# OettlM/STEDM

Measured on AMD Instinct MI355X. Metric: U-Net denoising steps/sec (32x32x4 latent, bs=64), higher is better.
Workload: dtype f16; 1 GPU; HER2-style DDIM-50 + CFG 1.5 (rescale 0.7) denoising step, NS32 U-Net (234.6M params, random-init PRNG weights), 32x32x4 latents + 3-ch layout concat, style vector 512; batch_per_gpu=64, global_batch=64, latent=32x32x4, cfg=cond+uncond per step, parallelism=dp1 (independent latents, no in-loop collective)

## Files before the change

include/stedm_hip.h:

```cpp
#ifndef STEDM_HIP_H
#define STEDM_HIP_H

#include <stdint.h>

#ifdef __cplusplus
extern "C" {
#endif

#define STEDM_ABI_VERSION 31

#define STEDM_F16 0
#define STEDM_BF16 1

#define STEDM_CONV_S1 0
#define STEDM_CONV_DOWN 1
#define STEDM_CONV_UP 2
#define STEDM_CONV_UP_SUBPIXEL 3
#define STEDM_CONV_S2D 4

int stedm_abi_version(void);
const char* stedm_last_error(void);
int stedm_device_cus(void);

#define STEDM_F16G_RAW 1
// ... 38 lines not shown
                           const float* gamma, const float* beta, float eps, int groups, int act, int B, int HW,
                           void* out_hi, void* out_lo, void* raw_hi, void* raw_lo, float* mean_rstd, const float* film, long film_bstride,
                           int film_off, int mm_dtype, void* stream);
int stedm_gn_apply16c_x16(int c1, const float* cs1, int nslab1, const float* x2, int c2, const float* cs2, int nslab2, int x2_bmod,
                          const float* gamma, const float* beta, float eps, int groups, int act, int B, int HW,
                          void* out_hi, void* raw_hi, int mm_dtype, void* stream);
int stedm_avgpool2x2(const float* in, float* out, int B, int H, int W, int C, float* chan_stats, int nslab, void* stream);
int stedm_replicate2x2(const float* in, float* out, int B, int H, int W, int C, float scale, int accumulate, float* chan_stats, int nslab,
                       void* stream);
int stedm_gn_apply16c_resample(const float* x, int C, const float* cs, int nslab, const float* gamma, const float* beta, float eps, int groups,
                               int act, int B, int H, int W, int mode, void* out_hi, void* out_lo, float* xr, float* mean_rstd, int mm_dtype,
                               void* stream);
int stedm_gn_stats(const float* x1, int c1, const float* x2, int c2, int x2_bmod, int groups, int B, int HW,
                   double* stats, void* stream);
int stedm_gn_apply16(const float* x1, int c1, const float* x2, int c2, int x2_bmod, const float* gamma,
                     const float* beta, float eps, int groups, int act, const double* stats, int B, int HW,
                     void* out_hi, void* out_lo, int mm_dtype, void* stream);

typedef struct stedm_conv_args {
  const float* src1;
  const float* src2;
  int32_t c1, c2, src2_bmod;
  int32_t B, Hin, Win;
  int32_t mode;
  int32_t ks;
  const float* scale;
  const float* shift;
  int32_t act;
  const void* w_hi;
  const void* w_lo;
  const float* bias;
  const float* emb;
  int32_t emb_bstride;
  const float* res;
  float* out;
  int32_t cout;
  int32_t npass;
  int32_t mm_dtype;
  const void* src16_hi;
  const void* src16_lo;
  int32_t act_out;
  void* out16_hi;
  void* out16_lo;
  const void* w_frag;
  float* chan_stats;
  const void* src16b_hi;
  const void* w_frag_b;
  const float* bias_b;
  int32_t cb;
  float* ws;
  int64_t ws_floats;
  int32_t chan_nslab;
  const void* w_frag16;
  const void* w_frag_b16;
  int32_t pad_br;
  const float* gn_gamma;
  const float* gn_beta;
  float gn_eps;
  int32_t gn_groups;
  int32_t gn_act;
  void* gn_out16;
  float* gn_mr;
  int32_t gn_only;
  void* gn_out16_lo;
  void* qkv_q;
  void* qkv_k;
  void* qkv_vt;
  int32_t qkv_T, qkv_Tp, qkv_heads;
  float qkv_qscale;
  const float* ln_gamma;
  const float* ln_beta;
  const float* ln_res;
  float ln_eps;
  int32_t out16_stride;
  void* gn_coop;
  const uint32_t* gn_coop_epoch;
  uint32_t* gn_coop_tmo;
  int32_t src16_cstride;
  int32_t k_chan0;
  int32_t w_cin;
  int32_t res_bmod;
  const float* res2;
  int32_t ws_bmod;
} stedm_conv_args;
int stedm_conv_igemm(const stedm_conv_args* args, void* stream);
int stedm_conv_fused_skip_ok(const stedm_conv_args* args);
int stedm_conv3x3_tiles_ok(int Hout, int Wout);
int stedm_im2col_rows16(const void* src16, void* dst16, int B, int Hs, int Ws, int C, int mode, void* stream);
int stedm_conv_rs_ok(const stedm_conv_args* args);
int stedm_conv_partials(const stedm_conv_args* args, int32_t* nshare, int dry, void* stream);
int stedm_conv_finish(const stedm_conv_args* args, int nshare, void* stream);

int stedm_conv_in(const float* x1, int c1, const float* x2, int c2, int x2_bmod, const float* w_oihw,
                  const float* bias, float* out, int B, int H, int W, int cout, float* chan_stats, void* stream);
int stedm_conv_out(const float* src, int c, const float* chan_stats, int nslab, const float* gamma, const float* beta,
                   float eps, int groups, const float* w_hwio, const float* bias, float* out, int B, int H, int W,
                   int cout, void* stream);

int stedm_time_embed(const int64_t* t, const float* freqs, const float* w0t, const float* b0,
                     const float* w2t, const float* b2, float* emb, float* ws, int B, int mc, int ted,
                     void* stream);
int stedm_time_embed_f32(const float* t, const float* freqs, const float* w0t, const float* b0,
                         const float* w2t, const float* b2, float* emb, float* ws, int B, int mc, int ted,
                         void* stream);
int stedm_emb_proj(const float* emb, const float* wt, const float* bias, float* out, int B, int k, int ntot,
                   void* stream);

int stedm_linear(const float* x, const float* wt, const float* bias, float* out, int B, int k, int n, int act_in,
                 int act_out, void* stream);

int stedm_attn_legacy(const float* qkv, float* out, int B, int T, int heads, int ch, void* stream);
int stedm_attn_legacy16(const void* qkv, int qkv_is16, void* out16, int B, int T, int heads, int ch, int mm_dtype, void* stream);
#define STEDM_ATTN_HEADS_FIRST 0
#define STEDM_ATTN_QKV_FIRST 1
int stedm_attn_qkv(const float* qkv, float* out, int B, int T, int heads, int ch, int order, void* stream);
int stedm_attn_qkv16(const void* qkv, int qkv_is16, void* out16, int B, int T, int heads, int ch, int mm_dtype, int order, void* stream);

int stedm_ddim_step(const float* x, const float* e_c, const float* e_u, const float* noise,
                    const float* coefs, const int32_t* step_idx, float cfg_scale, float rescale_phi,
                    float* x_prev, float* pred_x0, int B, int C, int H, int W, void* stream);
int stedm_ddim_step_ex(const float* x, const float* e_c, const float* e_u, const float* noise, const float* coefs, const int32_t* step_idx,
                       int n_iters, float cfg_scale, float rescale_phi, int draw, float temperature, float noise_dropout, long first_id,
                       unsigned long long seed, float* x_prev, float* pred_x0, float* eps_out, float* noise_out, int B, int C, int H, int W,
                       void* stream);
int stedm_ddim_step_rows(const float* x, const float* e_c, const float* e_u, const float* noise, const float* coefs,
                         const int32_t* step_idx, int n_iters, const float* scales, float rescale_phi, int draw, long first_id,
                         unsigned long long seed, float* x_prev, float* pred_x0, int B, int C, int H, int W, void* stream);
int stedm_step_advance(int32_t* step_idx, int delta, void* stream);
int stedm_step_set_t(const int64_t* ts_table, const int32_t* step_idx, int64_t* t_buf, int B, void* stream);
int stedm_step_set_t_f32(const float* ts_table, const int32_t* step_idx, float* t_buf, int B, void* stream);

#define STEDM_DPM_NCOEF 6
int stedm_dpm_step(float* x, const float* e_c, const float* e_u, float* x0_prev, float* pred_x0, const float* coefs,
                   const int32_t* step_idx, float cfg_scale, long n, void* stream);

#define STEDM_DPMU_NCOEF 24
#define STEDM_DPMU_ALL 0
#define STEDM_DPMU_MODEL 1
#define STEDM_DPMU_COMBINE 2
int stedm_dpm_update(float* x, float* base, const float* e_c, const float* e_u, float* slots, long slot_stride, float* pred_x0,
                     const float* rows, const int32_t* step_idx, float cfg_scale, int mode, long n, void* stream);
int stedm_dpm_threshold(float* slots, long slot_stride, const float* rows, const int32_t* step_idx, float max_val, int B, long n,
                        float* q_out, void* stream);

#define STEDM_PLMS_EULER 0
#define STEDM_PLMS_HEUN 1
#define STEDM_PLMS_MULTISTEP 2
int stedm_plms_step(float* x, const float* e_c, const float* e_u, float* ring, const float* coefs, const int32_t* step_idx,
                    int n_iters, int phase, float cfg_scale, float* pred_x0, float* x_tmp, long n, void* stream);

int stedm_svit_patch_embed(const float* img, int B, int ns, int H, int W, int patch, const float* ln_w,
                           const float* ln_b, float eps, const float* wt, const float* bias, const float* pos,
                           const float* cls, float* x, int dim, void* stream);
int stedm_svit_patch_ln16(const float* img, int B, int ns, int H, int W, int patch, const float* ln_w, const float* ln_b,
                          float eps, void* out_hi, void* out_lo, int mm_dtype, void* stream);
int stedm_svit_tok_place(const float* tok, const float* pos, const float* cls, float* x, int B, int ntok, int dim, void* stream);
int stedm_ln_apply16(const float* x, const float* gamma, const float* beta, float eps, void* out_hi, void* out_lo,
                     long rows, int dim, int mm_dtype, void* stream);
int stedm_qkv_pack(const void* qkv, int qkv_is16, float qscale, void* q_hi, void* q_lo, void* k_hi, void* k_lo, void* vt_hi,
                   void* vt_lo, int B, int T, int Tp, int heads, int mm_dtype, void* stream);
int stedm_lsa_flash(const void* q_hi, const void* q_lo, const void* k_hi, const void* k_lo, const void* vt_hi,
                    const void* vt_lo, void* out_hi, void* out_lo, int B, int T, int Tp, int heads, int npass,
                    int mm_dtype, void* stream);
int stedm_qkv_pack_mx8(const void* qkv, int qkv_is16, float qscale, void* q8, void* qs, void* k8, void* ks, void* vt8, void* vs, int B, int T,
                       int Tp, int heads, int mm_dtype, void* stream);
int stedm_lsa_flash_mx8(const void* q8, const void* qs, const void* k8, const void* ks, const void* vt8, const void* vs, void* out16, int B,
// ... 179 lines not shown
```

stedm_amd/_lib.py:

```python
from __future__ import annotations

import ctypes as C
import os

_HERE = os.path.dirname(os.path.abspath(__file__))
LIB_PATH = os.environ.get("STEDM_HIP_LIB") or os.path.join(_HERE, "libstedm_hip.so")

ABI_VERSION = 31
F16, BF16 = 0, 1
CONV_S1, CONV_DOWN, CONV_UP, CONV_UP_SUBPIXEL, CONV_S2D = 0, 1, 2, 3, 4
STREAM_POSTERIOR = 0x40000


class StedmHipError(RuntimeError):
    pass


class ConvArgs(C.Structure):
    _fields_ = [
        ("src1", C.c_void_p), ("src2", C.c_void_p),
        ("c1", C.c_int32), ("c2", C.c_int32), ("src2_bmod", C.c_int32),
        ("B", C.c_int32), ("Hin", C.c_int32), ("Win", C.c_int32),
        ("mode", C.c_int32), ("ks", C.c_int32),
        ("scale", C.c_void_p), ("shift", C.c_void_p),
        ("act", C.c_int32),
        ("w_hi", C.c_void_p), ("w_lo", C.c_void_p), ("bias", C.c_void_p),
        ("emb", C.c_void_p), ("emb_bstride", C.c_int32),
        ("res", C.c_void_p), ("out", C.c_void_p),
        ("cout", C.c_int32), ("npass", C.c_int32), ("mm_dtype", C.c_int32),
        ("src16_hi", C.c_void_p), ("src16_lo", C.c_void_p),
        ("act_out", C.c_int32), ("out16_hi", C.c_void_p), ("out16_lo", C.c_void_p),
        ("w_frag", C.c_void_p), ("chan_stats", C.c_void_p),
        ("src16b_hi", C.c_void_p), ("w_frag_b", C.c_void_p), ("bias_b", C.c_void_p), ("cb", C.c_int32),
        ("ws", C.c_void_p), ("ws_floats", C.c_int64), ("chan_nslab", C.c_int32), ("w_frag16", C.c_void_p), ("w_frag_b16", C.c_void_p), ("pad_br", C.c_int32),
        ("gn_gamma", C.c_void_p), ("gn_beta", C.c_void_p), ("gn_eps", C.c_float), ("gn_groups", C.c_int32), ("gn_act", C.c_int32), ("gn_out16", C.c_void_p), ("gn_mr", C.c_void_p), ("gn_only", C.c_int32),
        ("gn_out16_lo", C.c_void_p),
        ("qkv_q", C.c_void_p), ("qkv_k", C.c_void_p), ("qkv_vt", C.c_void_p),
        ("qkv_T", C.c_int32), ("qkv_Tp", C.c_int32), ("qkv_heads", C.c_int32), ("qkv_qscale", C.c_float),
        ("ln_gamma", C.c_void_p), ("ln_beta", C.c_void_p), ("ln_res", C.c_void_p), ("ln_eps", C.c_float),
        ("out16_stride", C.c_int32),
        ("gn_coop", C.c_void_p), ("gn_coop_epoch", C.c_void_p), ("gn_coop_tmo", C.c_void_p),
        ("src16_cstride", C.c_int32), ("k_chan0", C.c_int32), ("w_cin", C.c_int32), ("res_bmod", C.c_int32),
        ("res2", C.c_void_p), ("ws_bmod", C.c_int32),
    ]


_P, _I, _F = C.c_void_p, C.c_int, C.c_float
SIGNATURES = {
    "stedm_abi_version": (_I, []),
    "stedm_last_error": (C.c_char_p, []),
    "stedm_device_cus": (_I, []),
    "stedm_f16_guard_set": (_I, [_P]),
    "stedm_pack_conv_weight": (_I, [_P, _P, _P, _I, _I, _I, _I, _P]),
    "stedm_pack_conv_weight_up": (_I, [_P, _P, _P, _I, _I, _I, _P]),
    "stedm_pack_conv_weight_frag": (_I, [_P, _P, _I, _I, _I, _I, _P]),
    "stedm_pack_conv_weight_up_frag": (_I, [_P, _P, _I, _I, _I, _P]),
    "stedm_pack_conv_weight_frag16": (_I, [_P, C.c_long, C.c_long, _I, _P, _I, _I, _I, _I, _P]),
    "stedm_pack_conv_weight_frag16_hl": (_I, [_P, C.c_long, C.c_long, _I, _P, _I, _I, _I, _P]),
    "stedm_pack_conv_weight_frag16_hl1": (_I, [_P, C.c_long, C.c_long, _I, _P, _I, _I, _I, _P]),
    "stedm_pack_conv_weight_up_frag16_hl": (_I, [_P, _P, _I, _I, _I, _P]),
    "stedm_pack_conv_weight_s2d_frag16_hl": (_I, [_P, _P, _I, _I, _I, _I, _P]),
    "stedm_pack_conv_weight_s2d_frag": (_I, [_P, _P, _I, _I, _I, _I, _P]),
    "stedm_space_to_depth16": (_I, [_P, _I, _I, _I, _I, _P, _P, _I, _P]),
    "stedm_transpose_f32": (_I, [_P, _P, _I, _I, _P]),
    "stedm_gn_scale_shift": (_I, [_P, _I, _P, _I, _I, _P, _P, _F, _I, _I, _I, _P, _P, _P]),
    "stedm_gn_nslab": (_I, [_I, _I]),
    "stedm_gn_stats": (_I, [_P, _I, _P, _I, _I, _I, _I, _I, _P, _P]),
    "stedm_gn_apply16": (_I, [_P, _I, _P, _I, _I, _P, _P, _F, _I, _I, _P, _I, _I, _P, _P, _I, _P]),
    "stedm_gn_chan_nslab": (_I, [_I]),
    "stedm_gn_chan_stats": (_I, [_P, _I, _I, _I, _I, _P, _P]),
    "stedm_gn_chan_stats16": (_I, [_P, _I, _I, _I, _I, _P, _P, _P, _I, _P]),
    "stedm_gn_apply16c": (_I, [_P, _I, _P, _I, _P, _I, _P, _I, _I, _P, _P, _F, _I, _I, _I, _I, _P, _P, _P, _P, _I, _P]),
    "stedm_gn_apply16c_mr": (_I, [_P, _I, _P, _I, _P, _I, _P, _I, _I, _P, _P, _F, _I, _I, _I, _I, _P, _P, _P, _P, _P, _I, _P]),
    "stedm_conv3x3_tiles_ok": (_I, [_I, _I]),
    "stedm_im2col_rows16": (_I, [_P, _P, _I, _I, _I, _I, _I, _P]),
    "stedm_philox_normal": (_I, [_P, _I, _I, _P, _I, C.c_ulonglong, C.c_uint, _P]),
    "stedm_ddim_mask_blend": (_I, [_P, _P, _P, C.c_long, C.c_long, _P, _P, _P, _P, _P, _I, _I, _I, C.c_long, C.c_ulonglong, _P]),
    "stedm_ddpm_step": (_I, [_P, _P, _P, _P, _I, _I, _P, _P, C.c_long, C.c_long, _P, _P, _P, _P, _I, _I, _I, C.c_long,
                            C.c_ulonglong, C.c_ulonglong, _P]),
    "stedm_ddpm_step_ex": (_I, [_P, _P, _P, _P, _P, _I, _I, _P, _P, _F, _P, _I, _P, C.c_long, C.c_long, _P, _P, _P, _P, _P, _P, _P, _P,
                               _I, _I, _I, C.c_long, C.c_ulonglong, C.c_ulonglong, _P]),
    "stedm_gn_apply16c_film": (_I, [_P, _I, _P, _I, _P, _I, _P, _I, _I, _P, _P, _F, _I, _I, _I, _I, _P, _P, _P, _P, _P, _P, C.c_long, _I, _I, _P]),
    "stedm_gn_apply16c_drop": (_I, [_P, _I, _P, _I, _P, _I, _P, _I, _I, _P, _P, _F, _I, _I, _I, _I, _P, _P, _P, _P, _P, _I, _F, C.c_ulonglong, C.c_uint,
                                    C.c_uint, _P, _P]),
    "stedm_gn_apply16c_film_drop": (_I, [_P, _I, _P, _I, _P, _I, _P, _I, _I, _P, _P, _F, _I, _I, _I, _I, _P, _P, _P, _P, _P, _P, C.c_long, _I, _I, _F,
                                         C.c_ulonglong, C.c_uint, C.c_uint, _P, _P]),
    "stedm_gn_apply16c_x16": (_I, [_I, _P, _I, _P, _I, _P, _I, _I, _P, _P, _F, _I, _I, _I, _I, _P, _P, _I, _P]),
    "stedm_conv_igemm": (_I, [C.POINTER(ConvArgs), _P]),
    "stedm_conv_fused_skip_ok": (_I, [C.POINTER(ConvArgs)]),
    "stedm_conv_rs_ok": (_I, [C.POINTER(ConvArgs)]),
    "stedm_conv_partials": (_I, [C.POINTER(ConvArgs), C.POINTER(C.c_int32), _I, _P]),
    "stedm_conv_finish": (_I, [C.POINTER(ConvArgs), _I, _P]),
    "stedm_conv_in": (_I, [_P, _I, _P, _I, _I, _P, _P, _P, _I, _I, _I, _I, _P, _P]),
    "stedm_conv_out": (_I, [_P, _I, _P, _I, _P, _P, _F, _I, _P, _P, _P, _I, _I, _I, _I, _P]),
    "stedm_time_embed": (_I, [_P, _P, _P, _P, _P, _P, _P, _P, _I, _I, _I, _P]),
    "stedm_time_embed_f32": (_I, [_P, _P, _P, _P, _P, _P, _P, _P, _I, _I, _I, _P]),
    "stedm_emb_proj": (_I, [_P, _P, _P, _P, _I, _I, _I, _P]),
    "stedm_linear": (_I, [_P, _P, _P, _P, _I, _I, _I, _I, _I, _P]),
    "stedm_attn_legacy": (_I, [_P, _P, _I, _I, _I, _I, _P]),
    "stedm_attn_legacy16": (_I, [_P, _I, _P, _I, _I, _I, _I, _I, _P]),
    "stedm_attn_qkv": (_I, [_P, _P, _I, _I, _I, _I, _I, _P]),
    "stedm_attn_qkv16": (_I, [_P, _I, _P, _I, _I, _I, _I, _I, _I, _P]),
    "stedm_ddim_step": (_I, [_P, _P, _P, _P, _P, _P, _F, _F, _P, _P, _I, _I, _I, _I, _P]),
    "stedm_ddim_step_ex": (_I, [_P, _P, _P, _P, _P, _P, _I, _F, _F, _I, _F, _F, C.c_long, C.c_ulonglong, _P, _P, _P, _P, _I, _I, _I, _I,
                               _P]),
    "stedm_ddim_step_rows": (_I, [_P, _P, _P, _P, _P, _P, _I, _P, _F, _I, C.c_long, C.c_ulonglong, _P, _P, _I, _I, _I, _I, _P]),
    "stedm_step_advance": (_I, [_P, _I, _P]),
    "stedm_step_set_t": (_I, [_P, _P, _P, _I, _P]),
    "stedm_step_set_t_f32": (_I, [_P, _P, _P, _I, _P]),
    "stedm_dpm_step": (_I, [_P, _P, _P, _P, _P, _P, _P, _F, C.c_long, _P]),
    "stedm_dpm_update": (_I, [_P, _P, _P, _P, _P, C.c_long, _P, _P, _P, _F, _I, C.c_long, _P]),
    "stedm_dpm_threshold": (_I, [_P, C.c_long, _P, _P, _F, _I, C.c_long, _P, _P]),
    "stedm_plms_step": (_I, [_P, _P, _P, _P, _P, _P, _I, _I, _F, _P, _P, C.c_long, _P]),
    "stedm_svit_patch_embed": (_I, [_P, _I, _I, _I, _I, _I, _P, _P, _F, _P, _P, _P, _P, _P, _I, _P]),
    "stedm_svit_patch_ln16": (_I, [_P, _I, _I, _I, _I, _I, _P, _P, _F, _P, _P, _I, _P]),
    "stedm_svit_tok_place": (_I, [_P, _P, _P, _P, _I, _I, _I, _P]),
    "stedm_ln_apply16": (_I, [_P, _P, _P, _F, _P, _P, C.c_long, _I, _I, _P]),
    "stedm_qkv_pack": (_I, [_P, _I, _F, _P, _P, _P, _P, _P, _P, _I, _I, _I, _I, _I, _P]),
    "stedm_lsa_flash": (_I, [_P, _P, _P, _P, _P, _P, _P, _P, _I, _I, _I, _I, _I, _I, _P]),
    "stedm_lsa_flash_drop": (_I, [_P, _P, _P, _P, _P, _P, _P, _P, _I, _I, _I, _I, _I, _I, _F, C.c_ulonglong, C.c_uint, _P]),
    "stedm_dropout_rows": (_I, [_P, _P, _P, _P, _P, C.c_long, _F, C.c_ulonglong, C.c_uint, _I, _P]),
    "stedm_qkv_pack_mx8": (_I, [_P, _I, _F, _P, _P, _P, _P, _P, _P, _I, _I, _I, _I, _I, _P]),
    "stedm_lsa_flash_mx8": (_I, [_P, _P, _P, _P, _P, _P, _P, _I, _I, _I, _I, _I, _P]),
    "stedm_svit_head": (_I, [_P, _I, _I, _I, _I, _P, _P, _P, _F, _P, _P, _P, _I, _P, C.c_long, _P]),
    "stedm_lsa_bwd_ws_floats": (C.c_long, [_I, _I, _I, _I]),
    "stedm_lsa_bwd16_ws_bytes": (C.c_long, [_I, _I, _I, _I, _F]),
# ... 123 lines not shown
```

stedm_amd/csrc/conv_dma_bf16_p1.hip:

```cpp
#include "conv_igemm_dma9.inc"
#include "conv_rs.inc"
namespace stedm {
int conv_dma_pick_bf16_p1(ConvParams& p, hipStream_t st, bool dry) {
  int rc = conv_rs_pick<__bf16>(p, st, dry);
  if (rc >= 0 || dry || p.a.src16b_hi || p.a.mode == STEDM_CONV_S2D || p.a.qkv_q || p.a.ln_gamma) return rc;
  if (p.a.src16_cstride || p.a.k_chan0 || p.a.w_cin || p.a.res_bmod || p.a.res2 || p.partials || p.a.out16_stride) return rc;
  rc = dma9_pick<__bf16>(p, st);
  return rc >= 0 ? rc : dma_pick<1, __bf16>(p, st);
}
}

extern "C" int stedm_debug_conv_stamps(unsigned long long* host_out, int nblocks) {
  if (!host_out || nblocks <= 0 || nblocks > 2048) { stedm::set_error("debug_conv_stamps: bad args"); return 1; }
  hipError_t e = hipMemcpyFromSymbol(host_out, HIP_SYMBOL(g_conv_stamps), (size_t)nblocks * 8 * sizeof(unsigned long long));
  if (e != hipSuccess) { stedm::set_error("debug_conv_stamps: %s", hipGetErrorString(e)); return 2; }
  return 0;
}
```

stedm_amd/csrc/conv_dma_f16_p1.hip:

```cpp
#include "conv_igemm_dma9.inc"
#include "conv_rs.inc"
namespace stedm {
int conv_dma_pick_f16_p1(ConvParams& p, hipStream_t st, bool dry) {
  int rc = conv_rs_pick<_Float16>(p, st, dry);
  if (rc >= 0 || dry || p.a.src16b_hi || p.a.mode == STEDM_CONV_S2D || p.a.qkv_q || p.a.ln_gamma) return rc;
  if (p.a.src16_cstride || p.a.k_chan0 || p.a.w_cin || p.a.res_bmod || p.a.res2 || p.partials || p.a.out16_stride) return rc;
  rc = dma9_pick<_Float16>(p, st);
  return rc >= 0 ? rc : dma_pick<1, _Float16>(p, st);
}
int conv_splitk_finish(ConvParams& p, int nshare, hipStream_t st) { return splitk_finish_impl(p, nshare, st); }
}
```

stedm_amd/csrc/conv_igemm_dma.hip:

```cpp
#include "conv_common.hpp"
using namespace stedm;

namespace stedm {
int conv_dma_pick_f16_p1(ConvParams&, hipStream_t, bool dry);
int conv_dma_pick_f16_p3(ConvParams&, hipStream_t, bool dry);
int conv_dma_pick_bf16_p1(ConvParams&, hipStream_t, bool dry);
int conv_dma_pick_bf16_p3(ConvParams&, hipStream_t, bool dry);
}

int stedm::conv_launch_dma(ConvParams& p, hipStream_t st, bool dry) {
  const stedm_conv_args& a = p.a;
  if (a.src16b_hi && a.npass != 1) { set_error("conv_igemm(dma): the fused skip phase is single-product only"); return 1; }
  if (dry && a.npass != 1 && !a.w_frag16) return 1;
  if (a.src16b_hi && ((long)a.B * a.Hin * a.Win * a.cb >= (1L << 31) || a.cb * 2 + 256 > STEDM_ZERO_PAGE_BYTES)) {
    set_error("conv_igemm(dma): fused skip operand too large (cb=%d)", a.cb);
    return 1;
  }
  if ((long)a.B * a.Hin * a.Win * (p.cstride > p.Cin ? p.cstride : p.Cin) >= (1L << 31)) {
    set_error("conv_igemm(dma): activation tensor too large for 32-bit element offsets");
    return 1;
  }
  if (p.Cin * 2 + 256 > STEDM_ZERO_PAGE_BYTES) { set_error("conv_igemm(dma): Cin too large for the zero page"); return 1; }
  const bool f16 = a.mm_dtype == STEDM_F16;
  int rc = a.npass == 3 ? (f16 ? conv_dma_pick_f16_p3(p, st, dry) : conv_dma_pick_bf16_p3(p, st, dry))
                        : (f16 ? conv_dma_pick_f16_p1(p, st, dry) : conv_dma_pick_bf16_p1(p, st, dry));
  if (dry) return rc < 0 ? 1 : 0;
  if (rc < 0 && a.ln_gamma) { set_error("conv_igemm(dma): the register-streamed kernel does not run this LayerNorm-epilogue problem (see stedm_conv_rs_ok)"); return 1; }
  if (rc < 0 && a.qkv_q) { set_error("conv_igemm(dma): the register-streamed kernel does not run this qkv-epilogue problem (see stedm_conv_rs_ok)"); return 1; }
  if (rc < 0 && (a.src16_cstride || a.k_chan0 || a.w_cin || a.res_bmod || a.res2 || p.partials || a.out16_stride)) {
    set_error("conv_igemm(dma): the register-streamed kernel does not run this problem, and no other kernel knows a K window, res_bmod / res2, the partials-only form or out16_stride (see stedm_conv_rs_ok)");
    return 1;
  }
  if (rc < 0 && a.src16b_hi) { set_error("conv_igemm(dma): no kernel runs this fused skip problem (see stedm_conv_fused_skip_ok)"); return 1; }
  if (rc < 0) { set_error("conv_igemm(dma): no tile configuration fits (Hin=%d Win=%d mode=%d Cin=%d)", a.Hin, a.Win, a.mode, p.Cin); return 1; }
  return rc;
}
```

stedm_amd/csrc/conv_rs.inc:

```
#pragma once
#include <type_traits>

#include "conv_igemm_dma.inc"
#include "gn_fold.hpp"

static __device__ unsigned long long g_conv_stamps[2048 * 8];
#define STAMP(K) if (STEDM_DBG(p.dbg, 1024) && tid == 0 && blockIdx.x < 2048) g_conv_stamps[blockIdx.x * 8 + (K)] = wall_clock64()
#define STAMPC(K) if (STEDM_DBG(p.dbg, 1024) && tid == 0 && blockIdx.x < 2048) g_conv_stamps[blockIdx.x * 8 + (K)] = __builtin_amdgcn_s_memtime()

#ifdef STEDM_CONV_DIAG
#define RS_DIAG(BIT) ((STEDM_CONV_DIAG) & (BIT))
#else
#define RS_DIAG(BIT) 0
#endif

__device__ __forceinline__ float rs_lane_xor1(float v) {
  return __builtin_bit_cast(float, __builtin_amdgcn_mov_dpp(__builtin_bit_cast(int, v), 0xB1, 0xF, 0xF, true));
}
template <typename T>
__device__ __forceinline__ unsigned rs_pack2(float lo, float hi) {
  typedef T V2T __attribute__((ext_vector_type(2)));
  V2T v; v[0] = (T)lo; v[1] = (T)hi;
  return __builtin_bit_cast(unsigned, v);
}
// ... 204 lines not shown
    }                                                                          \
  }
   \
   \
#define LOAD_A3(BASE, TAP, F)                                                  \
  {                                                                            \
    unsigned a_, a2_;                                                          \
    asm volatile("v_add_u32 %0, %1, %2" : "=v"(a_) : "s"((BASE) + tapd[TAP]), "v"(aofs[F]));             \
    asm volatile("v_add_u32 %0, %1, %2" : "=v"(a2_) : "s"((BASE) + tapd[TAP] + a_half), "v"(aofs[F]));   \
    LDSR(ah[(F) & (NAR - 1)], a_);                                             \
    LDSR(al[(F) & (NAR - 1)], a2_);                                            \
  }
#define A3_AFTER(Q, WHAT)                                                                                          \
  {                                                                                                                \
    if ((Q) + 2 < 8) { WHAT(Acur, t, (Q) + 2) }                                                                    \
    else if (t + 1 < NS) { WHAT(Acur, t + 1, (Q) + 2 - 8) }                                                         \
    else { WHAT(Anext, 0, (Q) + 2 - 8) }                                                                           \
  }
#define A3_ADDR_HI(BASE, TAP, F) asm volatile("v_add_u32 %0, %1, %2" : "=v"(a_) : "s"((BASE) + tapd[TAP]), "v"(aofs[F]));
#define A3_ADDR_LO(BASE, TAP, F) asm volatile("v_add_u32 %0, %1, %2" : "=v"(a2_) : "s"((BASE) + tapd[TAP] + a_half), "v"(aofs[F]));
#define RS3_CHUNK(PAR)                                                                                             \
  _Pragma("unroll") for (int u = 0; u < NU; ++u) {                                                                 \
    const int t = u >> 1, hf = u & 1, sb = (t & 1) ^ (PAR);                                                        \
    if (u == NU - 1) __builtin_amdgcn_s_barrier();    \
    _Pragma("unroll") for (int i = 0; i < 4; ++i) {                                                                \
      const int R = hf * 4 + i;                             \
      _Pragma("unroll") for (int m = 0; m < 12; ++m) {                                                             \
        const int j = m & 3;                                                                                       \
        __builtin_amdgcn_sched_barrier(0);                                                                         \
        if (m < 4) acc[R][j] = MM<T>::mfma16(al[R & (NAR - 1)], bh[sb][j], acc[R][j]);                              \
        else if (m < 8) acc[R][j] = MM<T>::mfma16(ah[R & (NAR - 1)], bl[sb][j], acc[R][j]);                         \
        else acc[R][j] = MM<T>::mfma16(ah[R & (NAR - 1)], bh[sb][j], acc[R][j]);                                    \
        __builtin_amdgcn_sched_barrier(0);                                                                         \
        if (m == 0) { LDSR(ah[(R + 1) & (NAR - 1)], a_); }                                                          \
        else if (m == 1) { LDSR(al[(R + 1) & (NAR - 1)], a2_); }                                                    \
        if (R == 0 && m >= 4) {                                                                                    \
                        \
          if (m == 4) { int g_ = g0 + t + 1; g_ = g_ < gmax ? g_ : gmax; wcur = wq + ((size_t)(unsigned)g_ << 13) + voff; } \
          if (m < 8) bh[sb ^ 1][m - 4] = *reinterpret_cast<const V8*>(wcur + (m - 4) * 1024);                        \
          else bl[sb ^ 1][m - 8] = *reinterpret_cast<const V8*>(wcur + wlo + (m - 8) * 1024);                        \
        }                                                                                                          \
        if (m == 10) A3_AFTER(R, A3_ADDR_HI)                                                                        \
        else if (m == 11) A3_AFTER(R, A3_ADDR_LO)                                                                   \
      }                                                                                                            \
    }                                                                                                              \
  }
  const unsigned char* wcur = wq + voff;
  unsigned a_ = 0, a2_ = 0;
  LOAD_B3(0, 0)
  LOAD_B3(1, 1)
  __syncthreads();
  {
    const unsigned Afirst = A0 + abuf * a_buf;
#pragma unroll
    for (int f = 0; f < NAR; ++f) LOAD_A3(Afirst, 0, f)
    A3_ADDR_HI(Afirst, 0, 1)
    A3_ADDR_LO(Afirst, 0, 1)
  }
#define RS3_STEP(STEP, PAR)                                                                                        \
  {                                                                                                                \
    const unsigned Acur = A0 + abuf * a_buf;                                                                       \
    if (++abuf == NABUF) abuf = 0;                                                                                 \
                                       \
    const unsigned Anext = (STEP) + 1 < nchunks ? A0 + abuf * a_buf : Acur;                                        \
    const int g0 = (STEP) * NS;                                                                                    \
    RS3_CHUNK(PAR)                                                                                                 \
  }
  int step = 0;
  for (; step + 1 < nchunks; step += 2) {
    RS3_STEP(step, 0)
    RS3_STEP(step + 1, NS & 1)
  }
  if (step < nchunks) RS3_STEP(step, 0)
#undef RS3_STEP
#undef RS3_CHUNK
#undef A3_AFTER
#undef A3_ADDR_HI
#undef A3_ADDR_LO
#undef LOAD_A3
#undef LOAD_B3
#undef LDSR
}

template <typename T, int WM, int KIND, bool FUSE = false, bool P3 = false>
__global__ void __launch_bounds__((16 / WM + 2) * 64) conv_rs_kernel(const ConvParams p) {
  static_assert(!FUSE || KIND == RS_3X3 || KIND == RS_3X3M, "the fused skip phase belongs to the 3x3 kinds");
  static_assert(!P3 || ((KIND == RS_3X3M || KIND == RS_1X1M || KIND == RS_SUBM) && !FUSE), "the 3-product form exists for the plain 16x16x32 kinds");
  static_assert(KIND != RS_1X1M || (P3 && !FUSE && WM == 4), "RS_1X1M is a 3-product kind");
  static_assert(KIND != RS_SUBM || (!FUSE && WM == 4), "RS_SUBM: plain epilogues, one compute wave per SIMD");
  constexpr int NCW = 16 / WM, NT = (NCW + 2) * 64, BMT = 256;
  constexpr bool NPERS = KIND == RS_1X1N, IS1X1 = KIND == RS_1X1 || NPERS, SUBM = KIND == RS_SUBM, SUBPIX = KIND == RS_SUB || SUBM;
  constexpr bool G1 = KIND == RS_1X1M;
  constexpr bool M16 = KIND == RS_3X3M || G1 || SUBM;
  constexpr bool GEO1 = IS1X1 || G1;
  constexpr bool IS3X3 = KIND == RS_3X3 || KIND == RS_3X3M;
  constexpr bool RES2 = IS3X3 && !FUSE && !P3;
  constexpr int NS = IS3X3 ? 9 : (SUBM ? 4 : (SUBPIX ? 8 : (G1 ? 1 : 4)));
  constexpr int NPL = (SUBPIX || KIND == RS_3X3M) ? 2 : 1;
  constexpr int NTAB = IS3X3 ? 9 : 4;
  constexpr int BROW = IS1X1 ? 128 : (G1 ? 64 : 32);
  constexpr int CPP = BROW / 16, RPB = 16 / CPP, PPI = 64 / CPP;
  constexpr int BKC = M16 ? 32 : NS * 16 / (IS3X3 ? 9 : (SUBPIX ? 4 : 1));
  constexpr int TAPS = NTAB, NABUF = P3 ? 3 : 4;
  constexpr int SST = kStageStride;

  extern __shared__ __attribute__((aligned(16))) unsigned char smem[];
  const int nai = (p.NP + PPI - 1) / PPI;
  const int a_plane = nai * 1024;
  const int a_half = NPL * a_plane + (M16 ? 32 : 0);
  const int a_buf = P3 ? 2 * a_half : ((FUSE && NPL * a_plane < 32768) ? 32768 : a_half);
  const int pl_skew = (KIND == RS_3X3M || SUBM) ? 16 : 0;
  int* sM = reinterpret_cast<int*>(smem);
  int* sMb = sM + BMT;
  unsigned char* sA = reinterpret_cast<unsigned char*>(sMb + BMT);
  float* sStage = reinterpret_cast<float*>(sA);
  const int ring_bytes = NABUF * a_buf;
  int* sIdx = reinterpret_cast<int*>(sA + ring_bytes);

  const stedm_conv_args& a = p.a;
  const int tid = threadIdx.x;
  const int lane = tid & 63;
  const int wave = __builtin_amdgcn_readfirstlane(tid >> 6);
  const bool is_loader = wave >= NCW;
  const int ntile = p.tiles_m * p.tiles_n;
  const bool s2d = SUBPIX && a.mode == STEDM_CONV_S2D;
  const int parity = (SUBPIX && !s2d) ? (blockIdx.x / ntile) & 3 : 0;
  const bool split = (IS3X3 || SUBPIX || GEO1) && p.ksplit >= 2;
  const int kz = split ? ((SUBPIX && !s2d) ? blockIdx.x / (4 * ntile) : blockIdx.x / ntile) : 0;
  const int bid = (SUBPIX || split) ? blockIdx.x % ntile : blockIdx.x;
  const int py = parity >> 1, px = parity & 1;
  int tile_n = bid % p.tiles_n, tile_m = bid / p.tiles_n;
  if (p.xcd_m) {
    const int gm = p.xcd_m, gn = 8 / gm, x = bid & 7, j = bid >> 3, tn_x = p.tiles_n / gn;
    const int jm = j / tn_x;
    tile_n = (j - jm * tn_x) * gn + x / gm;
    tile_m = jm * gm + x % gm;
  }
  constexpr bool npers = NPERS;
  if (npers) { tile_m = bid / p.npers; tile_n = (bid % p.npers) * (p.tiles_n / p.npers); }
  if STEDM_DBG(p.dbg, 256) { tile_n = 0; tile_m = 0; }
  const int m0 = tile_m * BMT, n0 = tile_n * BN;
  const int nchunks_all = p.Cin / BKC;
  const int nchunks_w = p.w_cin / BKC;
  const int nsteps = split ? nchunks_all / p.ksplit : nchunks_all;
  const int cbeg = kz * nsteps;
  const int nsteps2_all = FUSE ? a.cb / 64 : 0;
  const int nsteps2 = split ? nsteps2_all / p.ksplit : nsteps2_all;
  const int c2beg = split ? kz * nsteps2 : 0;
  STAMP(0);

  int b0, yo0;
  if (p.whole) { b0 = tile_m * p.nsamp; yo0 = 0; }
  else { b0 = m0 / p.HWout; yo0 = (m0 - b0 * p.HWout) / p.Wout; }
  const int br = s2d ? a.pad_br : 0;
  const int x0 = p.wsplit ? (m0 - b0 * p.HWout) - yo0 * p.Wout : 0;
  const int srow0 = ((a.mode == STEDM_CONV_S1 || SUBPIX) ? yo0 - 1 : (yo0 - 1) >> 1) + br;
  static_assert(RS_3X3 == 0, "");

  auto div_hw = [&](int n) { return (int)__umulhi((unsigned)n, p.mg_hw); };
  auto div_w = [&](int n) { return (int)__umulhi((unsigned)n, p.mg_w); };
  auto div_pw = [&](int n) { return (int)__umulhi((unsigned)n, p.mg_pw); };
  auto div_prpw = [&](int n) { return (int)__umulhi((unsigned)n, p.mg_prpw); };
  const int rem0 = GEO1 ? m0 - (m0 / p.HWout) * p.HWout : 0;
  auto patch_pixel = [&](int pos) {
    int off = -1;
    if (pos < p.NP) {
      if (GEO1) { if (m0 + pos < p.M) off = m0 + pos; }
      else {
        const int s_ = div_prpw(pos), rem = pos - s_ * (p.PRs * p.PW);
        const int prow = div_pw(rem), pcol = rem - prow * p.PW;
        const int b = b0 + s_, sy = srow0 + prow, sx = x0 + pcol - 1 + br;
        if (b < a.B && sy >= 0 && sy < a.Hin && sx >= 0 && sx < a.Win) off = (b * a.Hin + sy) * a.Win + sx;
      }
    }
    return off;
  };
  constexpr int NTC = NCW * 64;
  if (!is_loader) {
  for (int ml = tid; ml < BMT; ml += NTC) {
    int s_ = 0, yl = 0, x = 0, y = 0;
    if (!GEO1) {
      if (p.whole) { s_ = div_hw(ml); const int rem = ml - s_ * p.HWout; yl = div_w(rem); x = rem - yl * p.Wout; y = yl; }
      else { yl = div_w(ml); x = ml - yl * p.Wout; y = yo0 + yl; }
    }
#pragma unroll
    for (int tap = 0; tap < (M16 ? 1 : TAPS); ++tap) {
      int pos;
      if (GEO1) pos = ml;
      else {
        const int dy = SUBPIX ? (tap >> 1) + py : tap / 3, dx = SUBPIX ? (tap & 1) + px : tap - (tap / 3) * 3;
        int prow, pcol;
        if (a.mode == STEDM_CONV_S1 || SUBPIX) { prow = yl + dy; pcol = x + dx; }
        else { prow = ((y + dy - 1) >> 1) - srow0; pcol = ((x + dx - 1) >> 1) + 1; }
        pos = (s_ * p.PRs + prow) * p.PW + pcol;
      }
      sIdx[tap * BMT + ml] = (pos * BROW) | (M16 ? 0 : ((((pos / RPB) % CPP) ^ (IS1X1 ? 2 * tap : 0)) << 24));
    }
  }
  for (int ml = tid; ml < BMT; ml += NTC) {
    int m, b;
    if (GEO1) { m = m0 + ml; b = (IS1X1 && a.qkv_q) ? m / a.qkv_T : m0 / p.HWout + div_hw(rem0 + ml); }
    else if (!p.whole) { m = m0 + ml; b = b0; }
    else { const int s_ = div_hw(ml); b = b0 + s_; m = b * p.HWout + (ml - s_ * p.HWout); }
    const bool okm = m < p.M;
    if (SUBPIX && !s2d && okm) {
      const int rem = m - b * p.HWout, y = div_w(rem), x = rem - y * p.Wout;
      m = (b * 2 * p.Hout + 2 * y + py) * (2 * p.Wout) + 2 * x + px;
    }
    sM[ml] = okm ? m : -1;
    sMb[ml] = b;
  }
  }
  if (is_loader) {
    bool early[3] = {false, false, false};
#define WAIT_VM(N) asm volatile("s_waitcnt vmcnt(" #N ")" ::: "memory")
    const int aw = wave - NCW;
    const uint16_t* a_hi = reinterpret_cast<const uint16_t*>(a.src16_hi);
    const uint16_t* zero16 = reinterpret_cast<const uint16_t*>(g_zero_page);
    const int nslots = (nai + 1 - aw) / 2;
    constexpr int MAXS = IS1X1 ? 16 : 13;
    const uint16_t* asrc[MAXS];
    const int lpos = lane / CPP, lphys = lane % CPP;
    const long lo_delta = P3 ? reinterpret_cast<const uint16_t*>(a.src16_lo) - a_hi : 0;
    unsigned zmask = 0;
#define LO_SRC(K) (asrc[K] + (((zmask >> (K)) & 1u) ? 0 : lo_delta))
#pragma unroll
    for (int k = 0; k < MAXS; ++k) {
      asrc[k] = zero16;
      if (k < nslots) {
        const int pos = (aw + 2 * k) * PPI + lpos;
        const int logical = M16 ? lphys : lphys ^ ((pos / RPB) % CPP);
        const int pix = patch_pixel(pos);
        asrc[k] = (pix >= 0 ? a_hi + (long)pix * p.cstride : zero16) + logical * 8;
        if (P3 && pix < 0) zmask |= 1u << k;
        if (!STEDM_DBG(p.dbg, 2)) {
#pragma unroll
          for (int pl = 0; pl < NPL; ++pl) {
            GLDS16(asrc[k] + (cbeg * NPL + pl) * (BROW / 2), sA + pl * (a_plane + pl_skew) + (aw + 2 * k) * 1024);
            if (P3) GLDS16(LO_SRC(k) + (cbeg * NPL + pl) * (BROW / 2), sA + a_half + pl * (a_plane + pl_skew) + (aw + 2 * k) * 1024);
          }
        }
      }
    }
    auto issue_a = [&](int chunk) {
      if STEDM_DBG(p.dbg, 2) return;
      unsigned char* dsta = sA + (chunk % NABUF) * a_buf;
#pragma unroll
      for (int pl = 0; pl < NPL; ++pl) {
        const int c0 = ((cbeg + chunk) * NPL + pl) * (BROW / 2);
#pragma unroll
        for (int k = 0; k < MAXS; ++k) {
          if (k < nslots) {
            GLDS16(asrc[k] + c0, dsta + pl * (a_plane + pl_skew) + (aw + 2 * k) * 1024);
            if (P3) GLDS16(LO_SRC(k) + c0, dsta + a_half + pl * (a_plane + pl_skew) + (aw + 2 * k) * 1024);
          }
        }
      }
    };
    if constexpr (P3) {
      if (nsteps > 1) issue_a(1);
      __syncthreads();
      WAIT_VM(0);
      __syncthreads();
      for (int s = 0; s < nsteps; ++s) {
        WAIT_VM(0);
        __builtin_amdgcn_s_barrier();
        if (s + 2 < nsteps) issue_a(s + 2);
      }
    } else {
    early[0] = true;
#pragma unroll
    for (int c = 1; c < 3; ++c)
      if (c < nsteps) { issue_a(c); early[c] = true; }
    __syncthreads();
    int aoff2[FUSE ? 16 : 1];
    if (FUSE) {
#pragma unroll
      for (int k = 0; k < 16; ++k) {
        const int ml = (aw + 2 * k) * 8 + (lane >> 3);
        const int logical = (lane & 7) ^ ((ml >> 1) & 7);
        const int m = sM[ml];
        aoff2[k] = m >= 0 ? m * a.cb + logical * 8 : -(logical * 8) - 1;
      }
    }
    auto issue2 = [&](int c2, int ringpos) {
      if STEDM_DBG(p.dbg, 2) return;
      const uint16_t* b_hi = reinterpret_cast<const uint16_t*>(a.src16b_hi);
      unsigned char* dsta = sA + ringpos * a_buf;
      const int c0 = (c2beg + c2) * 64;
#pragma unroll
      for (int k = 0; k < (FUSE ? 16 : 0); ++k) {
        const int o = aoff2[k];
        const uint16_t* sh = o >= 0 ? b_hi + o + c0 : zero16 + (-o - 1) + c0;
        GLDS16(sh, dsta + (aw + 2 * k) * 1024);
      }
    };
    auto issue_any = [&](int chunk) {
      if (!FUSE || chunk < nsteps) issue_a(chunk); else issue2(chunk - nsteps, chunk % NABUF);
    };
    const int ntot = nsteps + nsteps2;
    auto wait_keep = [&](int cnt) {
      switch (cnt) {
        case 1: WAIT_VM(1); break; case 2: WAIT_VM(2); break; case 3: WAIT_VM(3); break; case 4: WAIT_VM(4); break;
        case 5: WAIT_VM(5); break; case 6: WAIT_VM(6); break; case 7: WAIT_VM(7); break; case 8: WAIT_VM(8); break;
        case 9: WAIT_VM(9); break; case 10: WAIT_VM(10); break; case 11: WAIT_VM(11); break; case 12: WAIT_VM(12); break;
        case 13: WAIT_VM(13); break; case 14: WAIT_VM(14); break; case 15: WAIT_VM(15); break; case 16: WAIT_VM(16); break;
        case 18: WAIT_VM(18); break; case 20: WAIT_VM(20); break; case 22: WAIT_VM(22); break; case 24: WAIT_VM(24); break;
        default: WAIT_VM(0); break;
      }
    };
    auto wait_all_but = [&](int chunk) { wait_keep((FUSE && chunk >= nsteps) ? 16 : nslots * NPL); };
    {
      if (!early[0]) issue_any(0);
      if (ntot > 1 && !early[1]) issue_any(1);
      if (ntot > 2 && !early[2]) issue_any(2);
      if (ntot > 2 && !STEDM_DBG(p.dbg, 2)) wait_all_but(2); else WAIT_VM(0);
      __syncthreads();
      for (int s = 0; s < ntot; ++s) {
        if STEDM_DBG(p.dbg, 4) { if (s + 1 >= ntot) WAIT_VM(0); }
        else if (s + 2 < ntot && !STEDM_DBG(p.dbg, 2)) wait_all_but(s + 2); else WAIT_VM(0);
        if (!(M16 && RS_DIAG(32))) __builtin_amdgcn_s_barrier();
        if (s + 3 < ntot) issue_any(s + 3);
      }
    }
    }
    if (npers) return;
#undef LO_SRC
#undef WAIT_VM
  } else {
    __syncthreads();
    STAMP(1);
    STAMPC(2);
    const int wm = wave >> 1, wn = wave & 1;
    const int r = lane & 31, h = lane >> 5;
    const unsigned voff = lane * 16;
    int abuf = 0;
    const unsigned A0 = (unsigned)(uintptr_t)sA;
    if constexpr (M16) {
      const int r16 = lane & 15;
      unsigned aofs[1][8];
#pragma unroll
      for (int f = 0; f < 8; ++f) {
        const int e = sIdx[wm * 128 + f * 16 + r16];
        if (G1) aofs[0][f] = (unsigned)(e & 0xFFFFFF) + (unsigned)(lane >> 4) * 16u;
        else aofs[0][f] = (unsigned)(e & 0xFFFFFF) + (unsigned)h * 16u + (unsigned)((lane >> 4) & 1) * (unsigned)(a_plane + pl_skew);
      }
      unsigned tapd[NS];
#pragma unroll
      for (int t = 0; t < NS; ++t)
        tapd[t] = G1 ? 0u : (SUBM ? (unsigned)((t >> 1) * p.PW + (t & 1)) * 32u : (unsigned)((t / 3) * p.PW + (t % 3)) * 32u);
      const unsigned char* wq = reinterpret_cast<const unsigned char*>(a.w_frag16) +
                                (((((size_t)parity * p.tiles_n + tile_n) * nchunks_w + cbeg) * NS) * 8 + wn * 4) * 1024;
      f32x4 acc[8][4];
#pragma unroll
      for (int i = 0; i < 8; ++i)
#pragma unroll
        for (int j = 0; j < 4; ++j)
#pragma unroll
          for (int e = 0; e < 4; ++e) acc[i][j][e] = 0.f;
      if constexpr (P3) {
        const size_t wlo = (size_t)((SUBPIX && !s2d) ? 4 : 1) * p.tiles_n * nchunks_all * NS * 8 * 1024;
        rs_phase16_p3<T, NS, 2>(acc, aofs[0], tapd, A0, a_buf, (unsigned)a_half, abuf, nsteps, wq, wlo, voff);
      } else
      rs_phase16<T, NS, 1, true>(acc, aofs, tapd, A0, a_buf, abuf, nsteps, wq, voff, p.dbg);
      if (FUSE) {
        unsigned aofs2[2][8];
#pragma unroll
        for (int sl = 0; sl < 2; ++sl)
#pragma unroll
          for (int f = 0; f < 8; ++f) {
            const unsigned ml = wm * 128 + f * 16 + r16;
            aofs2[sl][f] = ml * 128 + ((((unsigned)(4 * sl) + (unsigned)(lane >> 4)) ^ ((ml >> 1) & 7)) << 4);
          }
        const unsigned tapd2[2] = {0u, 0u};
        const unsigned char* wq2 = reinterpret_cast<const unsigned char*>(a.w_frag_b16) + ((((size_t)tile_n * nsteps2_all + c2beg) * 2) * 8 + wn * 4) * 1024;
        rs_phase16<T, 2, 2, false>(acc, aofs2, tapd2, A0, a_buf, abuf, nsteps2, wq2, voff);
      }
      __syncthreads();
      STAMP(3);
      STAMPC(7);
      if (!STEDM_DBG(p.dbg, 64)) {
        const int g4 = lane >> 4;
#pragma unroll
        for (int i = 0; i < 8; ++i)
#pragma unroll
          for (int j = 0; j < 4; ++j) {
            float* dst = sStage + (wm * 128 + i * 16 + g4 * 4) * SST + wn * 64 + j * 16 + r16;
#pragma unroll
            for (int e = 0; e < 4; ++e) dst[e * SST] = acc[i][j][e];
          }
      }
    } else {
    unsigned aofs[TAPS][WM];
#pragma unroll
    for (int t = 0; t < TAPS; ++t)
#pragma unroll
      for (int i = 0; i < WM; ++i) {
        const int e = sIdx[t * BMT + wm * (WM * 32) + i * 32 + r];
        aofs[t][i] = (unsigned)(e & 0xFFFFFF) + ((((unsigned)e >> 24) ^ (unsigned)h) << 4);
      }
    const unsigned char* wq = reinterpret_cast<const unsigned char*>(a.w_frag) +
                              ((((size_t)parity * p.tiles_n + tile_n) * nchunks_w + cbeg) * NS * 4 + wn * 2) * 1024;

    f32x16 acc[WM][2];
    if constexpr (NPERS) {
      {
        const unsigned N = (unsigned)a.cout;
        const int HD = a.qkv_heads * 64, Tn = a.qkv_T;
        const unsigned Tp = (unsigned)a.qkv_Tp;
        const unsigned esz = a.out ? 4u : 2u;
        const unsigned out_bytes = STEDM_DBG(p.dbg, 2048) ? 0u : (unsigned)p.M * N * esz;
        const unsigned pl_bytes = (a.qkv_q && !STEDM_DBG(p.dbg, 2048)) ? (unsigned)(p.M / Tn) * (unsigned)HD * Tp * 2u : 0u;
        const auto rs_out = __builtin_amdgcn_make_buffer_rsrc(a.out ? (void*)a.out : a.out16_hi, 0, out_bytes, 0x00020000);
        const auto rs_res = __builtin_amdgcn_make_buffer_rsrc((void*)a.res, 0, a.res ? out_bytes : 0u, 0x00020000);
        const auto rs_q = __builtin_amdgcn_make_buffer_rsrc(a.qkv_q, 0, pl_bytes, 0x00020000);
        const auto rs_k = __builtin_amdgcn_make_buffer_rsrc(a.qkv_k, 0, pl_bytes, 0x00020000);
        const auto rs_v = __builtin_amdgcn_make_buffer_rsrc(a.qkv_vt, 0, pl_bytes, 0x00020000);
        const bool has_res = a.res != nullptr, gelu = a.act_out == 2;
        const float* __restrict__ bp = a.bias ? a.bias : reinterpret_cast<const float*>(g_zero_page);
        static_assert(STEDM_ZERO_PAGE_BYTES >= 4 * 8192, "the zero page stands in for a missing bias of up to 8192 channels");
        unsigned bad16 = 0u;
        const int rl0 = wm * 128 + 4 * h;
        const int tn_first = tile_n, tn_end = tile_n + p.tiles_n / p.npers;
        for (int tn = tn_first; tn < tn_end; ++tn) {
          const int n0t = tn * BN;
#pragma unroll
          for (int i = 0; i < WM; ++i)
#pragma unroll
            for (int j = 0; j < 2; ++j)
#pragma unroll
              for (int e = 0; e < 16; ++e) acc[i][j][e] = 0.f;
          const unsigned char* wqt = reinterpret_cast<const unsigned char*>(a.w_frag) + (((size_t)tn * nchunks_all) * NS * 4 + wn * 2) * 1024;
          const int sec = a.qkv_q ? n0t / HD : 0;
          abuf = 0;
          if (tn == tn_first) rs_phase<T, WM, NS, NTAB, true, true>(acc, aofs, A0, a_buf, a_plane, abuf, nsteps, wqt, voff, p.dbg);
          else if (sec == 2) rs_phase<T, WM, NS, NTAB, false, true, true, true>(acc, aofs, A0, a_buf, a_plane, abuf, nsteps, wqt, voff, p.dbg);
          else rs_phase<T, WM, NS, NTAB, false, true, true, false>(acc, aofs, A0, a_buf, a_plane, abuf, nsteps, wqt, voff, p.dbg);
          if (a.qkv_q) {
            if (sec == 2) {
              const int cb = n0t - 2 * HD + wn * 64 + 4 * h + (lane & 1);
              const bool odd = lane & 1;
#pragma unroll
              for (int i = 0; i < WM; ++i) {
                __builtin_amdgcn_sched_barrier(0);
                const int rl = wm * 128 + i * 32 + (r & ~1), m = m0 + rl;
                const int b = sMb[rl], t = m - b * Tn;
                const unsigned o0 = (((unsigned)b * (unsigned)HD + (unsigned)cb) * Tp + (unsigned)t) * 2u;
#pragma unroll
                for (int j = 0; j < 2; ++j)
#pragma unroll
                  for (int e = 0; e < 16; e += 2) {
                    const int c = j * 32 + 8 * (e >> 2) + (e & 3);
                    const float a0 = acc[i][j][e] + bp[n0t + wn * 64 + 4 * h + c], a1 = acc[i][j][e + 1] + bp[n0t + wn * 64 + 4 * h + c + 1];
                    const float recv = rs_lane_xor1(odd ? a0 : a1);
                    const unsigned pk = rs_pack2<T>(odd ? recv : a0, odd ? a1 : recv);
                    __builtin_amdgcn_raw_buffer_store_b32(pk, rs_v, o0 + (unsigned)c * Tp * 2u, 0, 0);
                    bad16 |= f16_over2<T>(pk);
                  }
              }
            } else {
              const float sc = sec == 0 ? a.qkv_qscale : 1.0f;
              const auto rs_qk = sec == 0 ? rs_q : rs_k;
              const bool odd = lane & 1;
              const int cl = n0t - sec * HD + wn * 64 + (odd ? 32 : 0) + (r & ~1);
              const float b0 = bp[n0t + wn * 64 + (odd ? 32 : 0) + (r & ~1)], b1 = bp[n0t + wn * 64 + (odd ? 32 : 0) + (r & ~1) + 1];
              const unsigned ocol = (unsigned)(cl >> 6) * Tp * 128u + (unsigned)(cl & 63) * 2u;
#pragma unroll
              for (int i = 0; i < WM; ++i)
#pragma unroll
                for (int q4 = 0; q4 < 4; ++q4) {
                  __builtin_amdgcn_sched_barrier(0);
                  const int rl = rl0 + i * 32 + 8 * q4;
                  const int4 b4 = *reinterpret_cast<const int4*>(sMb + rl);
// ... 30 lines not shown
                }
#pragma unroll
                for (int e = 0; e < 16; ++e) {
                  float v = acc[i][j][e] + bsv;
                  if (has_res) v += rv[e];
                  __builtin_amdgcn_raw_buffer_store_b32(__builtin_bit_cast(unsigned, v), rs_out, o0 + (unsigned)(8 * (e >> 2) + (e & 3)) * N * 4u, 0, 0);
                }
              }
          } else {
            auto store16 = [&](auto with_gelu) {
              const bool odd = lane & 1;
              const unsigned col = (unsigned)(n0t + wn * 64 + (odd ? 32 : 0) + (r & ~1));
              const bool cv = col < N;
              const float b0 = bp[cv ? col : 0u], b1 = bp[cv ? col + 1 : 0u];
#pragma unroll
              for (int i = 0; i < WM; ++i) {
                __builtin_amdgcn_sched_barrier(0);
                const unsigned o0 = cv ? ((unsigned)(m0 + rl0 + i * 32) * N + col) * 2u : 0x80000000u;
#pragma unroll
                for (int e = 0; e < 16; ++e) {
                  const float a0 = acc[i][0][e], a1 = acc[i][1][e];
                  const float recv = rs_lane_xor1(odd ? a0 : a1);
                  const float v0 = (odd ? recv : a0) + b0, v1 = (odd ? a1 : recv) + b1;
                  const unsigned pk = decltype(with_gelu)::value ? rs_pack2<T>(gelu_erf_f(v0), gelu_erf_f(v1)) : rs_pack2<T>(v0, v1);
                  __builtin_amdgcn_raw_buffer_store_b32(pk, rs_out, o0 + (unsigned)(8 * (e >> 2) + (e & 3)) * N * 2u, 0, 0);
                  bad16 |= f16_over2<T>(pk);
                }
              }
            };
            if (gelu) store16(std::true_type{}); else store16(std::false_type{});
          }
        }
        f16_guard_commit(p.ovf, bad16, STEDM_F16G_CONV_OUT16);
        return;
      }
    }
#pragma unroll
    for (int i = 0; i < WM; ++i)
#pragma unroll
      for (int j = 0; j < 2; ++j)
#pragma unroll
        for (int e = 0; e < 16; ++e) acc[i][j][e] = 0.f;

    rs_phase<T, WM, NS, NTAB, true, !IS3X3>(acc, aofs, A0, a_buf, a_plane, abuf, nsteps, wq, voff, p.dbg);
    if (FUSE) {
      unsigned aofs2[4][WM];
#pragma unroll
      for (int sl = 0; sl < 4; ++sl)
#pragma unroll
        for (int i = 0; i < WM; ++i) {
          const unsigned ml = wm * (WM * 32) + i * 32 + r;
          aofs2[sl][i] = ml * 128 + ((((2 * sl) ^ ((ml >> 1) & 7)) ^ (unsigned)h) << 4);
        }
      const unsigned char* wq2 = reinterpret_cast<const unsigned char*>(a.w_frag_b) + ((((size_t)tile_n * nsteps2_all + c2beg) * 4) * 4 + wn * 2) * 1024;
      rs_phase<T, WM, 4, 4, false>(acc, aofs2, A0, a_buf, 0, abuf, nsteps2, wq2, voff);
    }
    __syncthreads();
    STAMP(3);
    STAMPC(7);
    if (IS1X1 && a.qkv_q && n0 >= 2 * a.qkv_heads * 64) {
#pragma unroll
      for (int i = 0; i < WM; ++i)
#pragma unroll
        for (int j = 0; j < 2; ++j) {
          float* dst = sStage + (wn * 64 + j * 32 + r) * kStageStrideT + wm * (WM * 32) + i * 32 + 4 * h;
#pragma unroll
          for (int q4 = 0; q4 < 4; ++q4)
            *reinterpret_cast<float4*>(dst + 8 * q4) = make_float4(acc[i][j][4 * q4], acc[i][j][4 * q4 + 1], acc[i][j][4 * q4 + 2], acc[i][j][4 * q4 + 3]);
        }
    } else
    if (!STEDM_DBG(p.dbg, 64)) {
#pragma unroll
      for (int i = 0; i < WM; ++i)
#pragma unroll
        for (int j = 0; j < 2; ++j) {
          float* dst = sStage + (wm * (WM * 32) + i * 32 + 4 * h) * SST + wn * 64 + j * 32 + r;
#pragma unroll
          for (int e = 0; e < 16; ++e) dst[((e & 3) + 8 * (e >> 2)) * SST] = acc[i][j][e];
        }
    }
    }
  }
  if (is_loader) __syncthreads();
  if STEDM_DBG(p.dbg, 64) return;
  __syncthreads();
  STAMP(5);

  const bool vec_ok = (a.cout & 3) == 0;
  const int c4 = tid & 31, rg = tid >> 5;
  const int n = n0 + c4 * 4;
  const bool active = n < a.cout;
  const int nv = !active ? 0 : (vec_ok ? 4 : (a.cout - n < 4 ? a.cout - n : 4));
  float bv[4] = {0.f, 0.f, 0.f, 0.f};
  if (a.bias && !split) for (int u = 0; u < nv; ++u) bv[u] = a.bias[n + u];
  if (FUSE && a.bias_b && !split) for (int u = 0; u < nv; ++u) bv[u] += a.bias_b[n + u];
  if constexpr (IS1X1 && !NPERS) {
    if (a.ln_gamma) {
      typedef T V4T __attribute__((ext_vector_type(4)));
      const int c4l = tid & 31, nl = c4l * 4;
      const bool act = nl < a.cout;
      float4 gm = make_float4(0.f, 0.f, 0.f, 0.f), bt = gm, bs = gm;
      if (act) {
        gm = *reinterpret_cast<const float4*>(a.ln_gamma + nl); bt = *reinterpret_cast<const float4*>(a.ln_beta + nl);
        if (a.bias) bs = *reinterpret_cast<const float4*>(a.bias + nl);
      }
      const float inv_dim = 1.0f / (float)a.cout;
      const float* __restrict__ lres = a.ln_res;
      float* __restrict__ outp = a.out;
      T* __restrict__ o16 = reinterpret_cast<T*>(a.out16_hi);
      unsigned bad16 = 0u;
      constexpr int RB = 4;
      for (int row0 = tid >> 5; row0 < BMT; row0 += RB * (NT / 32)) {
        int mm[RB];
        float4 r4[RB], v[RB];
        float s1[RB], s2[RB];
#pragma unroll
        for (int k = 0; k < RB; ++k) {
          const int row = row0 + k * (NT / 32);
          mm[k] = row < BMT ? sM[row] : -1;
          r4[k] = make_float4(0.f, 0.f, 0.f, 0.f); v[k] = r4[k];
          if (mm[k] >= 0 && act) {
            if (lres) r4[k] = *reinterpret_cast<const float4*>(lres + (long)mm[k] * a.cout + nl);
            v[k] = *reinterpret_cast<const float4*>(sStage + row * SST + nl);
            v[k].x += bs.x; v[k].y += bs.y; v[k].z += bs.z; v[k].w += bs.w;
          }
          s1[k] = (v[k].x + v[k].y) + (v[k].z + v[k].w);
        }
#pragma unroll
        for (int ofs = 16; ofs > 0; ofs >>= 1)
#pragma unroll
          for (int k = 0; k < RB; ++k) s1[k] += __shfl_xor(s1[k], ofs, 64);
#pragma unroll
        for (int k = 0; k < RB; ++k) {
          const float mean = s1[k] * inv_dim;
          v[k].x = act ? v[k].x - mean : 0.f; v[k].y = act ? v[k].y - mean : 0.f; v[k].z = act ? v[k].z - mean : 0.f; v[k].w = act ? v[k].w - mean : 0.f;
          s2[k] = (v[k].x * v[k].x + v[k].y * v[k].y) + (v[k].z * v[k].z + v[k].w * v[k].w);
        }
#pragma unroll
        for (int ofs = 16; ofs > 0; ofs >>= 1)
#pragma unroll
          for (int k = 0; k < RB; ++k) s2[k] += __shfl_xor(s2[k], ofs, 64);
#pragma unroll
        for (int k = 0; k < RB; ++k) {
          if (mm[k] < 0 || !act) continue;
          const float rstd = 1.0f / sqrtf(s2[k] * inv_dim + a.ln_eps);
          const long o = (long)mm[k] * a.cout + nl;
          const float w0 = v[k].x * rstd * gm.x + bt.x + r4[k].x, w1 = v[k].y * rstd * gm.y + bt.y + r4[k].y;
          const float w2 = v[k].z * rstd * gm.z + bt.z + r4[k].z, w3 = v[k].w * rstd * gm.w + bt.w + r4[k].w;
          if (outp) *reinterpret_cast<float4*>(outp + o) = make_float4(w0, w1, w2, w3);
          if (o16) {
            V4T h4; h4[0] = (T)w0; h4[1] = (T)w1; h4[2] = (T)w2; h4[3] = (T)w3;
            *reinterpret_cast<V4T*>(o16 + o) = h4;
            bad16 |= f16_over_v4<T>(h4);
          }
        }
      }
      f16_guard_commit(p.ovf, bad16, STEDM_F16G_NORM);
      return;
    }
  }
  if constexpr (IS1X1) {
    if (a.qkv_q) {
      typedef T V8T __attribute__((ext_vector_type(8)));
      typedef T V2T __attribute__((ext_vector_type(2)));
      const int H = a.qkv_heads, HD = H * 64, sec = n0 / HD, Tn = a.qkv_T;
      const long Tp = a.qkv_Tp;
// ... 408 lines not shown
    const int cpg = C / a.gn_groups, ng = (QB * 4) / cpg;
    __syncthreads();
    if (t < ng) {
      double s_ = 0.0, q_ = 0.0;
      for (int c = t * cpg; c < (t + 1) * cpg; ++c) { s_ += (double)gsum[(c >> 2) * 8 + (c & 3)]; q_ += (double)gsum[(c >> 2) * 8 + 4 + (c & 3)]; }
      gn_mean_rstd(s_, q_, 1.0 / ((double)cpg * HW), a.gn_eps, gmr[t * 2], gmr[t * 2 + 1]);
      if (a.gn_mr) { float* d = a.gn_mr + ((long)b * a.gn_groups + (qb0 * 4) / cpg + t) * 2; d[0] = gmr[t * 2]; d[1] = gmr[t * 2 + 1]; }
    }
    __syncthreads();
    if (tp < npl) {
      const int g = (tq * 4) / cpg;
      const float mean = gmr[g * 2], rstd = gmr[g * 2 + 1];
      const float4 gm = *reinterpret_cast<const float4*>(a.gn_gamma + n), bt = *reinterpret_cast<const float4*>(a.gn_beta + n);
      const float4 sc = make_float4(rstd * gm.x, rstd * gm.y, rstd * gm.z, rstd * gm.w);
      for (int pix = px0 + tp; pix < px1; pix += npl) {
        const long o = ((long)b * HW + pix) * C + n;
        float4 w = *reinterpret_cast<const float4*>(a.out + o);
        w.x = (w.x - mean) * sc.x + bt.x; w.y = (w.y - mean) * sc.y + bt.y; w.z = (w.z - mean) * sc.z + bt.z; w.w = (w.w - mean) * sc.w + bt.w;
        if (a.gn_act == 1) { w.x = silu_f(w.x); w.y = silu_f(w.y); w.z = silu_f(w.z); w.w = silu_f(w.w); }
        if (a.mm_dtype == STEDM_F16) {
          f16x4 h4; h4[0] = (_Float16)w.x; h4[1] = (_Float16)w.y; h4[2] = (_Float16)w.z; h4[3] = (_Float16)w.w;
          *reinterpret_cast<f16x4*>(reinterpret_cast<_Float16*>(a.gn_out16) + o) = h4;
          badn |= f16_over_v4<_Float16>(h4);
          if (a.gn_out16_lo) {
            f16x4 l4; l4[0] = (_Float16)(w.x - (float)h4[0]); l4[1] = (_Float16)(w.y - (float)h4[1]); l4[2] = (_Float16)(w.z - (float)h4[2]); l4[3] = (_Float16)(w.w - (float)h4[3]);
            *reinterpret_cast<f16x4*>(reinterpret_cast<_Float16*>(a.gn_out16_lo) + o) = l4;
          }
        } else {
          bf16x4 h4; h4[0] = (__bf16)w.x; h4[1] = (__bf16)w.y; h4[2] = (__bf16)w.z; h4[3] = (__bf16)w.w;
          *reinterpret_cast<bf16x4*>(reinterpret_cast<__bf16*>(a.gn_out16) + o) = h4;
          if (a.gn_out16_lo) {
            bf16x4 l4; l4[0] = (__bf16)(w.x - (float)h4[0]); l4[1] = (__bf16)(w.y - (float)h4[1]); l4[2] = (__bf16)(w.z - (float)h4[2]); l4[3] = (__bf16)(w.w - (float)h4[3]);
            *reinterpret_cast<bf16x4*>(reinterpret_cast<__bf16*>(a.gn_out16_lo) + o) = l4;
          }
        }
      }
      f16_guard_commit(ovf, badn, STEDM_F16G_NORM);
    }
  }
}

static bool splitk_reduce_launch(ConvParams& p, const int HWo, const long plane, const int ksplit, bool stats, const bool fine_ok, const bool gn_ok, hipStream_t st) {
  int qbs = 64;
  while (qbs > 8 && (long)p.a.B * ((HWo + 255) / 256) * ((p.a.cout / 4 + qbs - 1) / qbs) < 256) qbs >>= 1;
  const int cpg = (p.a.gn_out16 && p.a.gn_groups > 0) ? p.a.cout / p.a.gn_groups : 0;
  const bool gn = cpg > 0 && p.a.out && HWo <= 256 && gn_ok && p.a.chan_stats && stats && (p.a.chan_nslab == 0 || p.a.chan_nslab == 1) && p.a.cout % 32 == 0 &&
                  cpg % 4 == 0 && 32 % cpg == 0;
  if (gn) qbs = 8;
  int slab_px = 256;
  if (!gn) {
    if (p.a.chan_stats && stats && fine_ok) slab_px = HWo / p.a.chan_nslab;
    else if (!p.a.chan_stats || !stats)
      while (slab_px > 16 && HWo % (slab_px / 2) == 0 && (long)p.a.B * ((HWo + slab_px - 1) / slab_px) * ((p.a.cout / 4 + 7) / 8) < 512) slab_px >>= 1;
    if (slab_px < 256) {
      qbs = 256 / (slab_px < 32 ? slab_px : 32);
      if (qbs > 64) qbs = 64;
    }
  }
  dim3 grid(p.a.B, (HWo + slab_px - 1) / slab_px, (p.a.cout / 4 + qbs - 1) / qbs);
  stedm_conv_args ra = p.a;
  if (!stats) ra.chan_stats = nullptr;
  if (gn) {
    if (ksplit == 2) conv_splitk_reduce_kernel<2, true><<<grid, 256, 0, st>>>(ra, HWo, plane, 2, qbs, p.ovf);
    else conv_splitk_reduce_kernel<16, true><<<grid, 256, 0, st>>>(ra, HWo, plane, ksplit, qbs, p.ovf);
    p.gn_done = 1;
  } else if (ksplit == 2) conv_splitk_reduce_kernel<2><<<grid, 256, 0, st>>>(ra, HWo, plane, 2, qbs, p.ovf, slab_px);
  else conv_splitk_reduce_kernel<16><<<grid, 256, 0, st>>>(ra, HWo, plane, ksplit, qbs, p.ovf, slab_px);
  return ra.chan_stats != nullptr;
}

static int splitk_finish_impl(ConvParams& p, const int nshare, hipStream_t st) {
  const stedm_conv_args& a = p.a;
  const int HW = a.Hin * a.Win, nrun = (HW + 255) / 256;
  const bool fine_ok = a.chan_nslab > 0 && HW % a.chan_nslab == 0 && HW / a.chan_nslab >= 8 && HW / a.chan_nslab <= 256;
  const bool stats = a.chan_stats && (a.chan_nslab == 0 || a.chan_nslab == nrun || fine_ok);
  const long plane = (long)(a.ws_bmod ? a.ws_bmod : a.B) * HW * a.cout;
  p.gn_done = 0;
  const bool wrote = splitk_reduce_launch(p, HW, plane, nshare, stats, fine_ok, true, st);
  STEDM_LAUNCH_CHECK();
  p.stats_done = wrote ? 1 : 0;
  return 0;
}

template <typename T, int WM, int KIND, bool FUSE = false, bool P3 = false>
static int conv_rs_try(ConvParams& p, const ConvParams& q, hipStream_t st, bool dry = false) {
  constexpr size_t LDS_MAX = 160 * 1024;
  constexpr int BMT = 256;
  constexpr bool G1 = KIND == RS_1X1M;
  constexpr bool SUBK = KIND == RS_SUB || KIND == RS_SUBM;
  constexpr bool M16 = KIND == RS_3X3M || G1 || KIND == RS_SUBM;
  constexpr bool K1 = KIND == RS_1X1 || KIND == RS_1X1N;
  constexpr int PPI = K1 ? 8 : (G1 ? 16 : 32), NPL = (SUBK || KIND == RS_3X3M) ? 2 : 1, NTAB = (KIND == RS_3X3 || KIND == RS_3X3M) ? 9 : 4;
  if ((KIND == RS_3X3M || G1) && q.a.mode != STEDM_CONV_S1) return -1;
  const size_t nai = (q.NP + PPI - 1) / PPI;
  if ((nai + 1) / 2 > (K1 ? 16 : 13)) return -1;
  bool stats = q.a.chan_stats != nullptr;
  if (stats && (K1 || G1) && !(BMT % q.HWout == 0 || q.HWout % BMT == 0)) stats = false;
  const bool s2d = SUBK && q.a.mode == STEDM_CONV_S2D;
  const int nrun = (q.HWout + 255) / 256;
  const int HWo = (SUBK && !s2d) ? 4 * q.HWout : q.HWout;
  const bool fine_ok = q.ksplit >= 2 && q.a.chan_nslab > 0 && HWo % q.a.chan_nslab == 0 && HWo / q.a.chan_nslab >= 8 && HWo / q.a.chan_nslab <= 256;
  if (stats && q.a.chan_nslab != 0 && q.a.chan_nslab != ((SUBK && !s2d) ? 4 * nrun : nrun) && !fine_ok) stats = false;
  if (stats && SUBK && !s2d && q.a.chan_nslab == 0) stats = false;
  if (stats && q.ksplit >= 2 && !fine_ok && q.a.chan_nslab != 0 && (HWo + 255) / 256 != q.a.chan_nslab) stats = false;
  size_t a_buf = NPL * nai * 1024 + (M16 ? 32 : 0);
  if (FUSE && a_buf < 32768) a_buf = 32768;
  if (P3) a_buf *= 2;
  const size_t ring = (P3 ? 3 : 4) * a_buf;
  const size_t loop = ring + (size_t)(M16 ? 1 : NTAB) * BMT * sizeof(int);
  const size_t staging = (size_t)BMT * kStageStride * sizeof(float) + (stats ? (size_t)((16 / WM + 2) * 2) * 128 * 2 * sizeof(float) + (128 + 32) * 2 * sizeof(float) : 0);
  const size_t lds = (size_t)2 * BMT * sizeof(int) + (loop > staging ? loop : staging);
  if (lds > LDS_MAX) return -1;
  auto magic = [](int d) { return (unsigned)((0x100000000ull + (unsigned)d - 1) / (unsigned)d); };
  const bool flat = (K1 || G1) && q.a.B == 1;
  if (((K1 || G1) && q.HWout >= 65536 && !flat) || q.PRs * q.PW >= 65536 || (!(K1 || G1) && (long)q.HWout * q.Wout >= (1l << 32))) return -1;
  if (KIND == RS_1X1N &&
      !(WM == 4 && !FUSE && flat && q.ksplit < 2 && q.Cin <= 256 && q.tiles_n >= 2 && q.a.cout % 8 == 0 && (long)q.tiles_m * 4 >= (long)stedm_device_cus() * 3 &&
        !q.a.chan_stats && !q.a.emb && !q.a.gn_out16 && !q.a.out16_lo && !q.a.ln_gamma &&
        (q.a.qkv_q || (long)q.tiles_m * 256 * q.a.cout * (q.a.out ? 4 : 2) < (q.a.cout % 128 ? (1l << 31) : (1l << 32))) &&
        (!q.a.qkv_q || ((long)q.tiles_m * 256 / q.a.qkv_T + 2) * q.a.qkv_heads * 64 * q.a.qkv_Tp * 2 < (1l << 32)) &&
        ((q.a.qkv_q && q.tiles_n >= 3) || (q.a.out && !q.a.out16_hi && !q.a.act_out) || (!q.a.out && q.a.out16_hi && !q.a.res && !q.a.qkv_q)) &&
        !getenv("STEDM_CONV_NO_NPERS")))
    return -1;
  if (q.a.ln_gamma && (KIND != RS_1X1 || q.tiles_n != 1 || q.ksplit >= 2)) return -1;
  if (!q.a.out && q.a.chan_stats && !stats) return -1;
  if (q.a.out16_stride && (KIND == RS_1X1N || P3)) return -1;
  const bool kwin = q.a.src16_cstride || q.a.k_chan0 || q.a.w_cin;
  if ((kwin || q.a.res_bmod || q.a.res2 || q.partials) && !((KIND == RS_3X3 || KIND == RS_3X3M) && !FUSE && !P3)) return -1;
  if (q.a.res2 && q.a.cout % 4 != 0) return -1;
  if (dry) { p.nshare = q.ksplit >= 2 ? q.ksplit : 1; return 0; }
  p = q;
  p.mg_hw = flat ? 0u : magic(p.HWout); p.mg_w = magic(p.Wout); p.mg_pw = magic(p.PW); p.mg_prpw = magic(p.PRs * p.PW);
  {
    const double abytes = (double)p.M * (p.Cin + (FUSE ? p.a.cb : 0)) * 2.0 * (P3 ? 2 : 1);
    const double wbytes = (double)p.a.cout * (p.Cin * p.taps + (FUSE ? p.a.cb : 0)) * 2.0 * (P3 ? 2 : 1);
    double best = abytes * (p.tiles_n < 8 ? p.tiles_n : 8) + wbytes;
    p.xcd_m = 0;
    if (p.tiles_n > 1)
      for (int gm = 8; gm >= 2; gm >>= 1) {
        const int gn = 8 / gm;
        if (p.tiles_m % gm != 0 || p.tiles_n % gn != 0) continue;
        const double cost = abytes * gn + wbytes * gm;
        if (cost < best * 0.97) { best = cost; p.xcd_m = gm; }
      }
  }
  {
    const stedm_conv_args& a_ = p.a;
    const int cpg = (a_.gn_out16 && a_.gn_groups > 0) ? a_.cout / a_.gn_groups : 0;
    p.gn_tile = (cpg > 0 && stats && q.ksplit < 2 && (KIND == RS_3X3 || KIND == RS_3X3M) && (!P3 || a_.gn_out16_lo) && p.HWout <= BMT && BMT % p.HWout == 0 &&
                 a_.cout % 128 == 0 && cpg % 4 == 0 && 128 % cpg == 0 && a_.out && !a_.out16_hi && !a_.act_out) ? 1 : 0;
  }
  p.gn_coop = 0;
  {
    const stedm_conv_args& a_ = p.a;
    const int cpg = (a_.gn_out16 && a_.gn_groups > 0) ? a_.cout / a_.gn_groups : 0;
    const int nt = p.HWout / BMT;
    static const bool off = getenv("STEDM_NO_GN_COOP") != nullptr;
    if (!p.gn_tile && !off && cpg > 0 && stats && q.ksplit < 2 && (KIND == RS_3X3 || KIND == RS_3X3M) && !FUSE && !P3 && p.HWout % BMT == 0 && nt >= 2 && nt <= 4 &&
        a_.cout == 128 && p.tiles_n == 1 && p.xcd_m == 0 && !p.whole && cpg % 4 == 0 && 128 % cpg == 0 && 256 % a_.gn_groups == 0 && a_.out && !a_.out16_hi && !a_.act_out &&
        a_.gn_coop && a_.gn_coop_epoch && a_.gn_coop_tmo && (size_t)lds + 4 * 128 * 2 * sizeof(float) <= LDS_MAX)
      p.gn_coop = nt;
  }
  p.npers = 0;
  if (KIND == RS_1X1N) {
    const long cus = stedm_device_cus() > 0 ? stedm_device_cus() : 256;
    auto cost = [&](int s_) { return ((long)p.tiles_m * s_ + cus - 1) / cus * (2 + p.tiles_n / s_); };
    p.npers = (p.tiles_n % 2 == 0 && p.tiles_n >= 4 && cost(2) < cost(1)) ? 2 : 1;
  }
  ConvParams kp = p;
  if (!stats) kp.a.chan_stats = nullptr;
  if (q.a.k_chan0) {
    kp.a.src16_hi = reinterpret_cast<const unsigned char*>(q.a.src16_hi) + (size_t)q.a.k_chan0 * 2;
    if (q.a.w_frag) kp.a.w_frag = reinterpret_cast<const unsigned char*>(q.a.w_frag) + (size_t)q.a.k_chan0 * 9 * 256;
    if (q.a.w_frag16) kp.a.w_frag16 = reinterpret_cast<const unsigned char*>(q.a.w_frag16) + (size_t)q.a.k_chan0 * 9 * 256;
  }
  auto k = conv_rs_kernel<T, WM, KIND, FUSE, P3>;
  const size_t lds_launch = lds + (p.gn_coop ? (size_t)4 * 128 * 2 * sizeof(float) : 0);
  static size_t lds_set = 0;
  if (lds_launch > lds_set) {
    hipError_t e = hipFuncSetAttribute(reinterpret_cast<const void*>(k), hipFuncAttributeMaxDynamicSharedMemorySize, (int)lds_launch);
    if (e != hipSuccess) { set_error("conv_igemm(rs): hipFuncSetAttribute(%zu) failed: %s", lds_launch, hipGetErrorString(e)); return 2; }
    lds_set = lds_launch;
  }
  if (kp.ksplit >= 2) kp.a.chan_stats = nullptr;
  k<<<p.npers ? p.tiles_m * p.npers : p.tiles_m * p.tiles_n * ((SUBK && !s2d) ? 4 : 1) * (kp.ksplit >= 2 ? kp.ksplit : 1), (16 / WM + 2) * 64, lds_launch, st>>>(kp);
  STEDM_LAUNCH_CHECK();
  p.nshare = kp.ksplit >= 2 ? kp.ksplit : 1;
  if (kp.ksplit >= 2 && !p.partials) {
    stats = splitk_reduce_launch(p, HWo, (long)p.a.B * HWo * p.a.cout, kp.ksplit, stats, fine_ok, !(SUBK && !s2d), st);
    STEDM_LAUNCH_CHECK();
  }
  if (p.partials) return 0;
  if (stats) p.stats_done = 1;
  if (p.gn_tile || p.gn_coop) p.gn_done = 1;
  return 0;
}

template <typename T>
static int conv_rs_pick(ConvParams& p, hipStream_t st, bool dry = false) {
  const stedm_conv_args& a = p.a;
  const bool fuse = a.src16b_hi != nullptr;
  if (fuse && (a.ks != 3 || a.mode != STEDM_CONV_S1 || !a.w_frag_b || a.cb <= 0 || a.cb % 64 != 0 || a.res)) return -1;
  if ((!a.w_frag && !a.w_frag16) || (a.act_out != 0 && a.act_out != 2) || a.npass != 1 || a.mode == STEDM_CONV_DOWN) return -1;
  const bool s2d = a.mode == STEDM_CONV_S2D;
  const bool sp = (a.mode == STEDM_CONV_UP_SUBPIXEL || s2d) && p.taps == 4 && p.Cin % 32 == 0;
  if (s2d && !sp) return -1;
  const bool k3 = a.ks == 3 && p.taps == 9 && p.Cin % 16 == 0, k1 = a.ks == 1 && p.Cin % 64 == 0;
  if (!k3 && !k1 && !sp) return -1;
  if (a.qkv_q && (!k1 || fuse || !a.w_frag)) return -1;
  if (a.ln_gamma && (!k1 || fuse || !a.w_frag || a.cout > 128)) return -1;
  static int cus = 0;
  if (cus == 0) { cus = stedm_device_cus(); if (cus <= 0) cus = 256; }
  ConvParams q = p;
  if (!conv_geometry(q, 256, true)) return -1;
  q.ksplit = 0;
  auto pick_split = [&](long tiles, int nchunks, int planes = 1, int nchunks2 = 0) {
    if (!a.ws || (!a.out && !a.out16_hi) || a.out16_lo || a.act_out || a.cout % 4 != 0 || (a.emb && a.emb_bstride % 4 != 0) || a.ln_gamma || a.qkv_q) return 0;
    const int minc = tiles * 16 <= cus ? 1 : (tiles * 8 <= cus ? 2 : 4);
    int best = 0;
    for (int ks = 2; ks <= 16; ks *= 2) {
      if (nchunks % ks != 0 || nchunks / ks < minc || a.ws_floats < (long)ks * planes * p.M * a.cout || nchunks2 % ks != 0) break;
      best = ks;
      if (tiles * ks * 4 >= (long)cus * 3) break;
    }
    return best;
  };
  const bool subm = sp && a.w_frag16 && !a.w_frag;
  if (s2d) {
    q.ksplit = (long)q.tiles_m * q.tiles_n * 4 < (long)cus * 3 ? pick_split((long)q.tiles_m * q.tiles_n, p.Cin / 32) : 0;
    if (subm) { const int rc = conv_rs_try<T, 4, RS_SUBM>(p, q, st, dry); if (rc >= 0 || !a.w_frag) return rc; }
    return a.w_frag ? conv_rs_try<T, 4, RS_SUB>(p, q, st, dry) : -1;
  }
  const bool m16 = k3 && a.mode == STEDM_CONV_S1 && a.w_frag16 && p.Cin % 32 == 0 && p.Cin >= 256 && (!fuse || a.w_frag_b16);
  if (!a.w_frag && !m16 && !subm) return -1;
  if (fuse && !m16 && !a.w_frag_b) return -1;
  if ((long)q.tiles_m * q.tiles_n * (sp ? 4 : 1) * 4 < (long)cus * 3) {
    const int ks = k3 ? pick_split((long)q.tiles_m * q.tiles_n, p.Cin / (m16 ? 32 : 16), 1, fuse ? a.cb / 64 : 0)
                 : (k1 && !fuse)      ? pick_split((long)q.tiles_m * q.tiles_n, p.Cin / 64)
                 : sp                 ? pick_split((long)q.tiles_m * q.tiles_n * 4, p.Cin / 32, 4) : 0;
    const bool half_ok = k1 && (long)q.tiles_m * q.tiles_n * 2 >= cus;
    if (ks == 0 && !half_ok) return -1;
    q.ksplit = ks;
  }
  if (fuse) {
    if (!k3) return -1;
    int rc = m16 ? conv_rs_try<T, 4, RS_3X3M, true>(p, q, st, dry) : -1;
    if (rc >= 0 || !a.w_frag || !a.w_frag_b) return rc;
    if (m16) q.ksplit = 0;
    return conv_rs_try<T, 4, RS_3X3, true>(p, q, st, dry);
  }
  if (sp) {
    if (subm) { const int rc = conv_rs_try<T, 4, RS_SUBM>(p, q, st, dry); if (rc >= 0 || !a.w_frag) return rc; }
    return a.w_frag ? conv_rs_try<T, 4, RS_SUB>(p, q, st, dry) : -1;
  }
  if (k1) {
    const int rc = conv_rs_try<T, 4, RS_1X1N>(p, q, st, dry);
    return rc >= 0 ? rc : conv_rs_try<T, 4, RS_1X1>(p, q, st, dry);
  }
  if (m16) { const int rc = conv_rs_try<T, 4, RS_3X3M>(p, q, st, dry); if (rc >= 0 || !a.w_frag) return rc; q.ksplit = 0; }
  return conv_rs_try<T, 4, RS_3X3>(p, q, st, dry);
}

template <typename T>
static int conv_rs3_pick(ConvParams& p, hipStream_t st, bool dry = false) {
  const stedm_conv_args& a = p.a;
  const bool k1 = a.ks == 1 && p.taps == 1;
  const bool s2d = a.mode == STEDM_CONV_S2D;
  const bool sp = (a.mode == STEDM_CONV_UP_SUBPIXEL || s2d) && a.ks == 3 && p.taps == 4;
  if (a.npass != 3 || !a.w_frag16 || !a.src16_lo || a.src16b_hi || !(sp || ((k1 || (a.ks == 3 && p.taps == 9)) && a.mode == STEDM_CONV_S1)) ||
      p.Cin % 32 != 0 || p.Cin < (k1 ? 64 : 128) || (a.act_out != 0 && a.act_out != 2))
    return -1;
  static int cus = 0;
  if (cus == 0) { cus = stedm_device_cus(); if (cus <= 0) cus = 256; }
  ConvParams q = p;
  if (!conv_geometry(q, 256, true)) return -1;
  q.ksplit = 0;
  const long tiles = (long)q.tiles_m * q.tiles_n * ((sp && !s2d) ? 4 : 1);
  if (tiles * 4 < (long)cus * 3) {
    const int nchunks = p.Cin / 32;
    int best = 0;
    if (a.ws && a.out && !a.out16_hi && !a.act_out && a.cout % 4 == 0 && !(a.emb && a.emb_bstride % 4 != 0) && !(sp && !s2d))
      for (int ks = 2; ks <= 16; ks *= 2) {
        if (nchunks % ks != 0 || nchunks / ks < 4 || a.ws_floats < (long)ks * p.M * a.cout) break;
        best = ks;
        if (tiles * ks * 4 >= (long)cus * 3) break;
      }
    if (best == 0 && tiles * 2 < cus) return -1;
    q.ksplit = best;
  }
  if (k1) return conv_rs_try<T, 4, RS_1X1M, false, true>(p, q, st, dry);
  if (sp) return conv_rs_try<T, 4, RS_SUBM, false, true>(p, q, st, dry);
  return conv_rs_try<T, 4, RS_3X3M, false, true>(p, q, st, dry);
}
```

stedm_amd/ops.py:

```python
from __future__ import annotations

import ctypes as C
from dataclasses import dataclass
from typing import Optional, Tuple

import torch

from . import _lib
from ._lib import BF16, CONV_DOWN, CONV_S1, CONV_S2D, CONV_UP, CONV_UP_SUBPIXEL, F16, STREAM_POSTERIOR, ConvArgs, check, lib


@dataclass(frozen=True)
class Precision:
    mm_dtype: int = F16
    npass: int = 3
    attn_fp8: bool = False

    @staticmethod
    def parse(name: str) -> "Precision":
        table = {"parity": Precision(F16, 3), "parity_bf16": Precision(BF16, 3),
                 "fast": Precision(F16, 1), "f16": Precision(F16, 1), "bf16": Precision(BF16, 1),
                 "fp8": Precision(BF16, 1, True), "bf16+fp8attn": Precision(BF16, 1, True)}
        if name not in table:
            raise ValueError(f"unknown precision {name!r}; choose from {sorted(table)}")
# ... 373 lines not shown
        return self.frag(w4, cin * ks * ks, ks * ks, False, cout, cin, ks, m16)

    def _build_table(self, idxs):
        import struct
        rec, blk = [], 0
        for i in idxs:
            (w, sn, sc, flip, cout, cin, taps, m16, out) = self.items[i]
            rec.append(struct.pack("<QQqqiiiiii", w.data_ptr(), out.data_ptr(), sn, sc, cout, cin, taps, flip, m16, blk))
            blk += pack_blocks(cout, cin, m16)
        if not rec:
            return None, 0, 0
        return torch.frombuffer(bytearray(b"".join(rec)), dtype=torch.uint8).to(self.items[0][0].device), blk, len(rec)

    def set_fused(self, idxs) -> None:
        self._fused = frozenset(idxs)
        self._rest = None
        self._fresh = None

    def mark_fresh(self, versions) -> None:
        self._fresh = versions

    def run(self, versions=None) -> None:
        if not self.items:
            return
        fresh, self._fresh = self._fresh, None
        if self._fused and versions is not None and fresh == versions:
            if self._rest is None:
                self._rest = self._build_table([i for i in range(len(self.items)) if i not in self._fused])
            table, blocks, n = self._rest
            if n:
                check(lib().stedm_pack_frag_multi(table.data_ptr(), n, blocks, self.prec.mm_dtype, _stream()), "stedm_pack_frag_multi")
            return
        if self._table is None:
            self._table, self._blocks, _ = self._build_table(range(len(self.items)))
        check(lib().stedm_pack_frag_multi(self._table.data_ptr(), len(self.items), self._blocks, self.prec.mm_dtype, _stream()), "stedm_pack_frag_multi")


def conv3x3_tiles_ok(Hout: int, Wout: int) -> bool:
    return bool(lib().stedm_conv3x3_tiles_ok(int(Hout), int(Wout)))


_GENERIC_COLS: dict = {}


def _conv3x3_generic(src16, w_hi, w_lo, out, *, prec: Precision, mode: int, **kw):
    assert kw.get("skip") is None, "the fused skip phase belongs to the tiled kernels (stedm_conv_fused_skip_ok says so)"
    B, H, W, C = src16[0].shape
    Ho, Wo = ((H - 1) // 2 + 1, (W - 1) // 2 + 1) if mode == CONV_DOWN else ((2 * H, 2 * W) if mode == CONV_UP else (H, W))
    cols = []
    for i, pl in enumerate(src16):
        if pl is None or (i == 1 and prec.npass != 3):
            cols.append(None)
            continue
        key = (pl.device, i, B, Ho, Wo, 9 * C)
        col = _GENERIC_COLS.get(key)
        if col is None:
            if len(_GENERIC_COLS) > 16:
                _GENERIC_COLS.clear()
            col = _GENERIC_COLS[key] = torch.empty((B, Ho, Wo, 9 * C), dtype=torch.int16, device=pl.device)
        check(lib().stedm_im2col_rows16(pl.data_ptr(), col.data_ptr(), B, H, W, C, {CONV_S1: 0, CONV_DOWN: 1, CONV_UP: 2}[mode], _stream()),
              "stedm_im2col_rows16")
        cols.append(col)
    if isinstance(w_hi, LazyPlanes):
        w_hi, w_lo = w_hi.get()
    cout = w_hi.shape[0]
    assert tuple(w_hi.shape) == (cout, 9, C), (tuple(w_hi.shape), cout, C)
    for k in ("w_frag", "w_frag16", "ks", "out16_stride", "cout"):
        kw.pop(k, None)
    return conv_igemm(None, w_hi.view(cout, 1, 9 * C), None if w_lo is None else w_lo.view(cout, 1, 9 * C), out, prec=prec, ks=1, mode=CONV_S1,
                      src16=(cols[0], cols[1]), **kw)


def conv_igemm(src1: Optional[torch.Tensor], w_hi: torch.Tensor, w_lo: Optional[torch.Tensor], out: torch.Tensor, *, prec: Precision,
               ks: int = 3, mode: int = CONV_S1, src2: Optional[torch.Tensor] = None, src2_bmod: int = 0,
               scale: Optional[torch.Tensor] = None, shift: Optional[torch.Tensor] = None, act: int = 0,
               bias: Optional[torch.Tensor] = None, emb: Optional[torch.Tensor] = None, emb_offset: int = 0,
               emb_bstride: int = 0, res: Optional[torch.Tensor] = None,
               src16: Optional[Tuple[torch.Tensor, Optional[torch.Tensor]]] = None, act_out: int = 0,
               out16: Optional[Tuple[torch.Tensor, Optional[torch.Tensor]]] = None, w_frag: Optional[torch.Tensor] = None,
               chan_stats: Optional[torch.Tensor] = None,
               skip: Optional[Tuple[torch.Tensor, torch.Tensor, Optional[torch.Tensor]]] = None, query_fused: bool = False, query_rs: bool = False,
               ws: Optional[torch.Tensor] = None, pad_br: bool = False, w_frag16: Optional[torch.Tensor] = None,
               gn_next: Optional[tuple] = None, qkv_planes: Optional[tuple] = None, ln_after: Optional[tuple] = None, coop: Optional[tuple] = None,
               out16_stride: int = 0, cout: Optional[int] = None, res_bmod: int = 0, res2: Optional[torch.Tensor] = None, partials: bool = False):
    if src16 is not None and src1 is None and ks == 3 and mode in (CONV_S1, CONV_DOWN, CONV_UP) and not out16_stride:
        _, H_, W_, _ = src16[0].shape
        Ho_, Wo_ = ((H_ - 1) // 2 + 1, (W_ - 1) // 2 + 1) if mode == CONV_DOWN else ((2 * H_, 2 * W_) if mode == CONV_UP else (H_, W_))
        if not conv3x3_tiles_ok(Ho_, Wo_):
            if query_fused or query_rs:
                return False
            if not src16[0].is_contiguous() or res_bmod or res2 is not None or partials:
                raise _lib.StedmHipError("conv_igemm: a K window / res_bmod belongs to the tiled register-streamed kernel; this output grid takes the im2col form")
            return _conv3x3_generic(src16, w_hi, w_lo, out, prec=prec, mode=mode, scale=scale, shift=shift, act=act, bias=bias, emb=emb,
                                    emb_offset=emb_offset, emb_bstride=emb_bstride, res=res, act_out=act_out, out16=out16, chan_stats=chan_stats,
                                    skip=skip, ws=ws, gn_next=gn_next)
    if out is not None:
        _chk(out, name="out")
    a = ConvArgs()
    a.act_out = act_out
    if gn_next is not None:
        g_w, g_b, g_eps, g_groups, g_act, g_out = gn_next[:6]
        g_lo = None
        if isinstance(g_out, (tuple, list)):
            g_out, g_lo = g_out[0], g_out[1]
        g_mr = gn_next[6] if len(gn_next) > 6 else None
        a.gn_only = int(bool(gn_next[7])) if len(gn_next) > 7 else 0
        if g_mr is not None:
            _chk(g_mr, name="gn mean_rstd")
            assert tuple(g_mr.shape) == (out.shape[0], int(g_groups), 2)
            a.gn_mr = g_mr.data_ptr()
        _chk(g_w, name="gn gamma"); _chk(g_b, name="gn beta")
        assert g_out.dtype == torch.int16 and g_out.is_contiguous() and tuple(g_out.shape) == tuple(out.shape) and chan_stats is not None
        assert src16 is None or all(t is None or t.data_ptr() != g_out.data_ptr() for t in src16), "gn_next planes alias the convolution's input planes"
        a.gn_gamma, a.gn_beta, a.gn_eps, a.gn_groups, a.gn_act, a.gn_out16 = g_w.data_ptr(), g_b.data_ptr(), float(g_eps), int(g_groups), int(g_act), g_out.data_ptr()
        if g_lo is not None:
            assert g_lo.dtype == torch.int16 and g_lo.is_contiguous() and tuple(g_lo.shape) == tuple(out.shape)
            assert src16 is None or all(t is None or t.data_ptr() != g_lo.data_ptr() for t in src16), "gn_next lo planes alias the convolution's input planes"
            a.gn_out16_lo = g_lo.data_ptr()
        assert prec.npass == 1 or g_lo is not None, "gn_next in a 3-product mode needs the (hi, lo) planes"
        if coop is not None:
            cwd, cw = coop
            assert cwd.dtype == torch.int64 and cwd.is_contiguous() and tuple(cwd.shape) == (out.shape[0], 4, 128, 2)
            assert cw.dtype == torch.int32 and cw.numel() >= 2
            a.gn_coop, a.gn_coop_epoch, a.gn_coop_tmo = cwd.data_ptr(), cw.data_ptr(), cw.data_ptr() + 4
    a.pad_br = int(pad_br)
    a.w_frag16 = _ptr(w_frag16)
    a.w_frag = _ptr(w_frag) if prec.npass == 1 else None
    a.chan_stats = _ptr(chan_stats)
    a.chan_nslab = 0 if chan_stats is None else chan_stats.shape[1]
    if ws is not None:
        a.ws = ws.data_ptr()
        a.ws_floats = ws.numel()
    if skip is not None:
        a.src16b_hi = skip[0].data_ptr()
        a.cb = skip[0].shape[-1]
        a.w_frag_b = skip[1].data_ptr()
        a.bias_b = _ptr(skip[2])
        a.w_frag_b16 = _ptr(skip[3]) if len(skip) > 3 and prec.npass == 1 else None
    if out16 is not None:
        a.out16_hi = out16[0].data_ptr()
        a.out16_lo = _ptr(out16[1]) if prec.npass == 3 else None
        if out16_stride:
            assert cout is not None and out is None and prec.npass == 1 and out16[0].shape[-1] == out16_stride and out16[0].is_contiguous()
            a.out16_stride = int(out16_stride)
    if ln_after is not None:
        l_g, l_b, l_eps, l_res = ln_after
        _chk(l_g, name="ln gamma"); _chk(l_b, name="ln beta")
        assert res is None and prec.npass == 1 and (out is not None or out16 is not None)
        a.ln_gamma, a.ln_beta, a.ln_eps = l_g.data_ptr(), l_b.data_ptr(), float(l_eps)
        if l_res is not None:
            _chk(l_res, name="ln residual")
            a.ln_res = l_res.data_ptr()
    if qkv_planes is not None:
        qq, qk, qv, qT, qTp, qH, qs = qkv_planes
        assert out is None and out16 is None and prec.npass == 1 and src16 is not None
        nb = src16[0].shape[2] // int(qT)
        for t_, shp in ((qq, (nb * qH, qTp, 64)), (qk, (nb * qH, qTp, 64)), (qv, (nb * qH, 64, qTp))):
            assert t_.dtype == torch.int16 and t_.is_contiguous() and tuple(t_.shape) == shp, (tuple(t_.shape), shp)
        a.qkv_q, a.qkv_k, a.qkv_vt = qq.data_ptr(), qk.data_ptr(), qv.data_ptr()
        a.qkv_T, a.qkv_Tp, a.qkv_heads, a.qkv_qscale = int(qT), int(qTp), int(qH), float(qs)
        oshape = (1, 1, src16[0].shape[2], 3 * int(qH) * 64)
    else:
        oshape = out.shape if out is not None else out16[0].shape
        if cout is not None:
            oshape = tuple(oshape[:-1]) + (int(cout),)
    if src1 is not None:
        _chk(src1, name="src1")
        B, Hin, Win, c1 = src1.shape
        a.src1 = src1.data_ptr()
        a.src2 = _ptr(src2)
        c2 = 0 if src2 is None else src2.shape[-1]
    else:
        B, Hin, Win, c1 = src16[0].shape
        c2 = 0
    kwin = False
    if src16 is not None:
        s16 = src16[0]
        assert s16.dtype == torch.int16 and tuple(s16.shape) == (B, Hin, Win, c1 + c2)
        a.src16_hi = s16.data_ptr()
        a.src16_lo = _ptr(src16[1]) if prec.npass == 3 else None
        if not s16.is_contiguous():
            cs = s16.stride(2)
            base = s16._base if s16._base is not None else s16
            k0 = (s16.storage_offset() - base.storage_offset()) % cs
            assert src1 is None and tuple(s16.stride()) == (Hin * Win * cs, Win * cs, cs, 1) and k0 + c1 <= cs, \
                "src16[0] must be contiguous or a view plane[b0:b1, :, :, k0:k1] of a contiguous plane"
            assert cs % 32 == 0 and k0 % 32 == 0 and c1 % 32 == 0, "a K window is cut on 32-channel boundaries"
            kwin = True
            a.src16_hi = s16.data_ptr() - 2 * k0
            if a.src16_lo is not None:
                assert tuple(src16[1].stride()) == tuple(s16.stride()) and src16[1].storage_offset() == s16.storage_offset()
                a.src16_lo = src16[1].data_ptr() - 2 * k0
            a.src16_cstride, a.k_chan0 = cs, k0
            wplanes = w_hi._val[0] if isinstance(w_hi, LazyPlanes) and w_hi._val is not None else (None if isinstance(w_hi, LazyPlanes) else w_hi)
            a.w_cin = (w_frag.shape[-5] * 16 if w_frag is not None and prec.npass == 1 else
                       w_frag16.shape[-5] * 32 if w_frag16 is not None else wplanes.shape[-1] if wplanes is not None else cs)
            assert w_frag is None or w_frag16 is None or w_frag.shape[-5] * 16 == w_frag16.shape[-5] * 32
    a.res_bmod = int(res_bmod)
    if res_bmod:
        assert res is not None and res.is_contiguous() and res.dtype == torch.float32 and B % res_bmod == 0 and res.shape[0] >= res_bmod
    if res2 is not None:
        assert res is not None and res2.is_contiguous() and res2.dtype == torch.float32 and tuple(res2.shape) == tuple(res.shape)
        a.res2 = res2.data_ptr()
    a.c1, a.c2, a.src2_bmod = c1, c2, src2_bmod
    a.B, a.Hin, a.Win = B, Hin, Win
    a.mode, a.ks = mode, ks
    a.scale, a.shift, a.act = _ptr(scale), _ptr(shift), act
    lazy = w_hi if isinstance(w_hi, LazyPlanes) else None
    if lazy is not None:
        w_hi, w_lo = lazy._val if lazy._val is not None else (w_frag if w_frag is not None else w_frag16, None)
    a.w_hi, a.w_lo = _ptr(w_hi), (_ptr(w_lo) if prec.npass == 3 else None)
    a.bias = _ptr(bias)
    a.emb = None if emb is None else emb.data_ptr() + 4 * emb_offset
    a.emb_bstride = emb_bstride
    a.res = _ptr(res)
    a.out = _ptr(out)
    a.cout = oshape[-1]
    a.npass, a.mm_dtype = prec.npass, prec.mm_dtype
    if lazy is not None and lazy._val is None:
        if src16 is None or (w_frag is None and w_frag16 is None) or prec.npass != 1 or not lib().stedm_conv_rs_ok(C.byref(a)):
            w_hi, w_lo = lazy.get()
            a.w_hi, a.w_lo = _ptr(w_hi), (_ptr(w_lo) if prec.npass == 3 else None)
    elif mode == CONV_UP_SUBPIXEL:
        assert w_hi.shape == (4 * a.cout, 4, a.c1 + a.c2), (w_hi.shape, a.cout, a.c1, a.c2)
    elif mode == CONV_S2D:
        assert w_hi is None and (w_frag is not None or w_frag16 is not None) and src1 is None, \
            "the space-to-depth form runs on the register-streamed kernel only"
    else:
        assert w_hi.shape == (a.cout, ks * ks, a.w_cin if kwin else a.c1 + a.c2), (w_hi.shape, a.cout, ks, a.c1, a.c2)
    if partials:
        assert ws is not None and not query_fused
        n = C.c_int32(0)
        rc = lib().stedm_conv_partials(C.byref(a), C.byref(n), int(bool(query_rs)), _stream())
        if query_rs:
            return int(n.value) if rc == 0 else 0
        check(rc, "stedm_conv_partials")
        return int(n.value)
    if query_fused:
        return bool(lib().stedm_conv_fused_skip_ok(C.byref(a)))
    if query_rs:
        return bool(lib().stedm_conv_rs_ok(C.byref(a)))
    check(lib().stedm_conv_igemm(C.byref(a), _stream()), "stedm_conv_igemm")
    return out


def conv_finish(ws: torch.Tensor, nshare: int, out: Optional[torch.Tensor], *, prec: Precision, ws_bmod: int = 0, bias: Optional[torch.Tensor] = None,
                emb: Optional[torch.Tensor] = None, emb_offset: int = 0, emb_bstride: int = 0, res: Optional[torch.Tensor] = None,
                res2: Optional[torch.Tensor] = None, res_bmod: int = 0, chan_stats: Optional[torch.Tensor] = None,
                out16: Optional[Tuple[torch.Tensor, Optional[torch.Tensor]]] = None, out16_stride: int = 0, cout: Optional[int] = None,
                gn_next: Optional[tuple] = None):
    shape = tuple(out.shape) if out is not None else tuple(out16[0].shape[:-1]) + (int(cout),)
    B, H, W, co = shape
    a = ConvArgs()
    _chk(ws, name="ws")
    a.ws, a.ws_floats, a.ws_bmod = ws.data_ptr(), ws.numel(), int(ws_bmod)
    a.B, a.Hin, a.Win, a.cout = B, H, W, co
    a.mode, a.ks, a.npass, a.mm_dtype = CONV_S1, 3, prec.npass, prec.mm_dtype
    if out is not None:
        _chk(out, name="out")
        a.out = out.data_ptr()
    a.bias = _ptr(bias)
    if bias is not None:
        assert bias.numel() == co
    if emb is not None:
        assert emb.dtype == torch.float32 and emb.numel() >= emb_offset + (B - 1) * emb_bstride + co
        a.emb = emb.data_ptr() + 4 * emb_offset
    a.emb_bstride = int(emb_bstride)
    for r in (res, res2):
        if r is not None:
            _chk(r, name="res")
            assert tuple(r.shape[1:]) == (H, W, co) and r.shape[0] >= (res_bmod or B)
    assert res2 is None or res is not None
    a.res, a.res2, a.res_bmod = _ptr(res), _ptr(res2), int(res_bmod)
    if chan_stats is not None:
        _chk(chan_stats, name="chan_stats")
        assert chan_stats.shape[0] == B and tuple(chan_stats.shape[2:]) == (co, 2)
        a.chan_stats, a.chan_nslab = chan_stats.data_ptr(), chan_stats.shape[1]
    if out16 is not None:
        assert out16[0].dtype == torch.int16 and out16[0].is_contiguous() and tuple(out16[0].shape) == (B, H, W, out16_stride or co)
        a.out16_hi, a.out16_stride = out16[0].data_ptr(), int(out16_stride)
    if gn_next is not None:
        g_w, g_b, g_eps, g_groups, g_act, g_out = gn_next[:6]
        g_lo = None
        if isinstance(g_out, (tuple, list)):
            g_out, g_lo = g_out[0], g_out[1]
        g_mr = gn_next[6] if len(gn_next) > 6 else None
        _chk(g_w, name="gn gamma"); _chk(g_b, name="gn beta")
        assert out is not None and chan_stats is not None and g_out.dtype == torch.int16 and g_out.is_contiguous() and tuple(g_out.shape) == shape
        a.gn_gamma, a.gn_beta, a.gn_eps, a.gn_groups, a.gn_act, a.gn_out16 = g_w.data_ptr(), g_b.data_ptr(), float(g_eps), int(g_groups), int(g_act), g_out.data_ptr()
        if g_lo is not None:
            assert g_lo.dtype == torch.int16 and g_lo.is_contiguous() and tuple(g_lo.shape) == shape
            a.gn_out16_lo = g_lo.data_ptr()
        if g_mr is not None:
            _chk(g_mr, name="gn mean_rstd")
            assert tuple(g_mr.shape) == (B, int(g_groups), 2)
            a.gn_mr = g_mr.data_ptr()
    check(lib().stedm_conv_finish(C.byref(a), int(nshare), _stream()), "stedm_conv_finish")
    return out


def conv_in(x1: torch.Tensor, x2: Optional[torch.Tensor], w: torch.Tensor, bias: Optional[torch.Tensor], out: torch.Tensor,
# ... 1238 lines not shown
```

stedm_amd/unet.py:

```python
from __future__ import annotations

import math
import os
from typing import Dict, List, Optional, Tuple

import torch
import torch.nn as nn

from . import ops
from ._lib import BF16, F16, CONV_S2D, CONV_DOWN, CONV_S1, CONV_UP, CONV_UP_SUBPIXEL, StedmHipError
from .ops import Precision


def zero_module(module: nn.Module) -> nn.Module:
    for p in module.parameters():
        p.detach().zero_()
    return module


class GroupNorm32(nn.GroupNorm):
    """util.py:214-216 (container; eps 1e-5, 32 groups)."""


class TimestepBlock(nn.Module):
# ... 151 lines not shown
        self.dtype = torch.float32
        self.num_heads = num_heads
        self.num_head_channels = num_head_channels
        self.num_heads_upsample = num_heads_upsample
        self.predict_codebook_ids = False
        self.use_scale_shift_norm = bool(use_scale_shift_norm)
        ssn = self.use_scale_shift_norm
        self.precision = Precision.parse(precision) if isinstance(precision, str) else precision

        ted = model_channels * 4
        self.time_embed = nn.Sequential(nn.Linear(model_channels, ted), nn.SiLU(), nn.Linear(ted, ted))
        self.input_blocks = nn.ModuleList([TimestepEmbedSequential(nn.Conv2d(in_channels, model_channels, 3, padding=1))])
        input_block_chans = [model_channels]
        ch, ds = model_channels, 1
        for level, mult in enumerate(channel_mult):
            for _ in range(num_res_blocks):
                if ds in attention_resolutions:
                    raise TypeError("list.append() takes exactly one argument (0 given) "
                                    "[reference openaimodel.py:580: ds in attention_resolutions is not constructible]")
                self.input_blocks.append(TimestepEmbedSequential(ResBlock(ch, ted, dropout, out_channels=mult * model_channels,
                                                                                  use_scale_shift_norm=ssn)))
                ch = mult * model_channels
                input_block_chans.append(ch)
            if level != len(channel_mult) - 1:
                self.input_blocks.append(TimestepEmbedSequential(
                    ResBlock(ch, ted, dropout, out_channels=ch, use_scale_shift_norm=ssn, down=True) if resblock_updown
                    else Downsample(ch, conv_resample, out_channels=ch)))
                input_block_chans.append(ch)
                ds *= 2
        if num_head_channels != -1:
            num_heads = ch // num_head_channels
        dim_head = ch // num_heads if use_spatial_transformer else num_head_channels
        if use_spatial_transformer:
            from .attention import SpatialTransformer
            mid_attn = SpatialTransformer(ch, num_heads, dim_head, depth=transformer_depth, context_dim=context_dim)
        else:
            mid_attn = AttentionBlock(ch, num_heads=num_heads, num_head_channels=dim_head, use_new_attention_order=use_new_attention_order)
        self.middle_block = TimestepEmbedSequential(
            ResBlock(ch, ted, dropout, use_scale_shift_norm=ssn),
            ResBlockStyle(ch, ted, dropout, use_scale_shift_norm=ssn),
            mid_attn,
            ResBlock(ch, ted, dropout, use_scale_shift_norm=ssn),
        )
        self.output_blocks = nn.ModuleList([])
        for level, mult in list(enumerate(channel_mult))[::-1]:
            for i in range(num_res_blocks + 1):
                ich = input_block_chans.pop()
                layers: List[nn.Module] = [ResBlock(ch + ich, ted, dropout, out_channels=model_channels * mult, use_scale_shift_norm=ssn)]
                ch = model_channels * mult
                if ds in attention_resolutions:
                    raise TypeError("reference output block with ds in attention_resolutions is not runnable (openaimodel.py:689-698)")
                if level and i == num_res_blocks:
                    layers.append(ResBlock(ch, ted, dropout, out_channels=ch, use_scale_shift_norm=ssn, up=True) if resblock_updown
                                  else Upsample(ch, conv_resample, out_channels=ch))
                    ds //= 2
                self.output_blocks.append(TimestepEmbedSequential(*layers))
        self.out = nn.Sequential(GroupNorm32(32, ch), nn.SiLU(), zero_module(nn.Conv2d(model_channels, out_channels, 3, padding=1)))
        for k, rb in enumerate(self._all_resblocks()):
            rb.drop_site = k
        self.dropout_seed: Optional[int] = None
        self._drop_ctr: Optional[torch.Tensor] = None
        self._drop_step = 0
        self._drop_used: Dict[int, tuple] = {}
        self.last_dropout: Optional[Tuple[int, int]] = None

        self._packed: Dict[int, _Packed] = {}
        self._pack_key = None
        self._bufs: Dict[Tuple, torch.Tensor] = {}
        self._emb_layout: List[Tuple[ResBlock, int]] = []
        self._consts: Dict[str, torch.Tensor] = {}
        self._m16 = True
        self._gn_slot = 0
        self._style_cache: Dict[Tuple, torch.Tensor] = {}
        self._cs: Dict[int, torch.Tensor] = {}
        self._raw16: Dict[int, Tuple] = {}
        self._saved16: Dict = {}
        self._saved_mr: Dict = {}
        self._mr_ctr = 0
        self._plane_ctr = 0
        self._tape: Optional[list] = None
        self.cfg_shared_skip: Optional[bool] = None
        self.cfg_shared_front: Optional[bool] = None
        self.cfg_skip_partials: Optional[bool] = None

    def convert_to_fp16(self):
        pass

    def convert_to_fp32(self):
        pass

    def set_precision(self, precision) -> None:
        self.precision = Precision.parse(precision) if isinstance(precision, str) else precision
        self.invalidate()

    def invalidate(self) -> None:
        self._style_cache.clear()
        self._consts.clear()
        self._pack_key = None
        self._values_gen = getattr(self, "_values_gen", 0) + 1

    def check_f16_range(self, where: str = "UNetModel.forward") -> None:
        ops.f16_guard_check(where)

    def freshness_token(self, versions=None):
        if versions is None:
            versions = tuple(p._version for p in self.parameters())
        return (versions, getattr(self, "_values_gen", 0), ops.raw_write_epoch())

    def _buf(self, name: str, shape, dtype=torch.float32) -> torch.Tensor:
        key = (name, tuple(shape), dtype)
        t = self._bufs.get(key)
        if t is None:
            dev = next(self.parameters()).device
            t = torch.empty(tuple(shape), dtype=dtype, device=dev)
            self._bufs[key] = t
        return t

    def _timestep_blocks(self) -> List[ResBlock]:
        out = []
        for blk in list(self.input_blocks) + [self.middle_block] + list(self.output_blocks):
            for layer in blk:
                if isinstance(layer, ResBlock):
                    out.append(layer)
        return out

    def _all_resblocks(self) -> List[ResBlock]:
        out = []
        for blk in list(self.input_blocks) + [self.middle_block] + list(self.output_blocks):
            for layer in blk:
                if isinstance(layer, ResBlock):
                    out.append(layer)
                elif isinstance(layer, ResBlockStyle):
                    out.append(layer.block)
        return out

    @staticmethod
    def _drop_live(rb: ResBlock) -> bool:
        return bool(rb.training and rb.dropout > 0)

    def dropout_live(self) -> bool:
        return self.dropout > 0 and any(self._drop_live(rb) for rb in self._all_resblocks())

    @staticmethod
    def rank_dropout_seed(seed: int, rank: int) -> int:
        return (int(seed) ^ ((int(rank) * 0x9E3779B97F4A7C15) & 0xFFFFFFFFFFFFFFFF)) & 0xFFFFFFFFFFFFFFFF

    def set_dropout_step(self, step: int) -> None:
        dev = next(self.parameters()).device
        step = int(step) & 0xFFFFFFFF
        if self._drop_ctr is None or self._drop_ctr.device != dev:
            self._drop_ctr = torch.zeros((1,), dtype=torch.int32, device=dev)
        self._drop_ctr.fill_(step - (1 << 32) if step >= (1 << 31) else step)
        self._drop_step = step

    def _dropout_seed_now(self) -> int:
        if self.dropout_seed is None:
            self.dropout_seed = int(torch.randint(0, 2 ** 62, (1,), dtype=torch.int64).item())
        return self.dropout_seed

    def _dropout_begin(self) -> None:
        import torch.distributed as dist
        if self._drop_ctr is None or self._drop_ctr.device != next(self.parameters()).device:
            self.set_dropout_step(self._drop_step)
        seed = self._dropout_seed_now()
        rank = dist.get_rank() if dist.is_available() and dist.is_initialized() else 0
        ops.step_advance(self._drop_ctr, 1)
# ... 134 lines not shown
    def _splitk_ws_res(self, nel: int) -> Optional[torch.Tensor]:
        if nel > (1 << 23):
            return None
        return self._buf("conv_ws", ((16 if nel <= (1 << 20) else (4 if nel <= (1 << 22) else 2)) * nel,))

    def _splitk_ws(self, nel: int) -> torch.Tensor:
        return self._buf("conv_ws", ((16 if nel <= (1 << 20) else 2) * nel,))

    def _cs_new(self, t: torch.Tensor, nslab: Optional[int] = None) -> torch.Tensor:
        B, C = t.shape[0], t.shape[-1]
        HW = t.numel() // (B * C)
        cs = self._buf(f"cs.{t.data_ptr()}", (B, nslab or ops.gn_chan_nslab(HW), C, 2))
        self._cs[t.data_ptr()] = cs
        return cs

    def _chan_stats(self, t: torch.Tensor) -> torch.Tensor:
        cs = self._cs.get(t.data_ptr())
        if cs is None:
            cs = self._cs_new(t)
            ops.gn_chan_stats(t, cs)
        return cs

    def _norm16(self, norm: Optional[nn.GroupNorm], act: int, x1, x2=None, x2_bmod=0, want_raw=False):
        B, H, W, _ = x1.shape
        C = x1.shape[-1] + (0 if x2 is None else x2.shape[-1])
        pre = self._pre16.pop(x1.data_ptr(), None) if self._pre16 else None
        if pre is not None and norm is not None and pre[0] == id(norm) and pre[1] == act and x2 is None and not want_raw and self._tape is None:
            return pre[2]
        x16 = self._x16.pop(x1.data_ptr(), None)
        if x16 is not None:
            rawp, c1 = x16
            assert norm is not None and want_raw and tuple(rawp.shape) == (B, H, W, C) and c1 == x1.shape[-1]
            hi = self._planes(B, H, W, C)[0]
            ops.gn_apply16c_x16(c1, self._cs[x1.data_ptr()], x2, None if x2 is None else self._chan_stats(x2), hi, rawp, self.precision,
                                norm.weight, norm.bias, norm.eps, norm.num_groups, act, x2_bmod)
            return (hi, None), (rawp, None)
        if norm is None:
            hi, lo = self._planes(B, H, W, C)
            ops.gn_apply16(x1, x2, hi, lo, self.precision, x2_bmod=x2_bmod)
            return hi, lo
        (hi, lo), raw, mr = self._keep(norm, x1, (B, H, W, C), want_raw=want_raw)
        self._gn_site(norm, act, x1, x2, x2_bmod, hi=hi, lo=lo, prec=self.precision, raw=raw, mean_rstd=mr)
        return ((hi, lo), raw) if want_raw else (hi, lo)

    def _keep(self, norm: nn.GroupNorm, x, shape, kind="a16", want_raw=False):
        B, H, W, C = shape
        key = (id(norm), x.data_ptr())
        keep = self._tape is not None and self.precision.npass == 1 and self.precision.mm_dtype == BF16
        if keep:
            self._plane_ctr += 1
            planes = self._saved16[key] = self._planes(B, H, W, C, f"keep{self._plane_ctr}.a16")
        else:
            planes = self._planes(B, H, W, C, kind)
        raw = None
        if want_raw and keep:
            raw = self._saved16[("raw", x.data_ptr())] = self._planes(B, H, W, C, f"keep{self._plane_ctr}.raw16")
        elif want_raw:
            raw = self._planes(B, H, W, C, "raw16")
        mr = None
        if self._tape is not None:
            self._mr_ctr += 1
            mr = self._saved_mr[key] = self._buf(f"keep{self._mr_ctr}.mr", (B, norm.num_groups, 2))
        return planes, raw, mr

    def _gn_site(self, norm: nn.GroupNorm, act: int, x1, x2=None, x2_bmod=0, *, hi, lo, prec, raw=None, mean_rstd=None, film=None, film_off=0,
                 film_bstride=0, drop=None, resample=0, xr=None) -> None:
        w, b, eps, G = norm.weight, norm.bias, norm.eps, norm.num_groups
        if resample:
            assert x2 is None and film is None and drop is None and raw is None
            ops.gn_apply16c_resample(x1, self._chan_stats(x1), hi, lo, prec, w, b, resample, eps, G, act, xr=xr, mean_rstd=mean_rstd)
        elif drop is not None:
            ops.gn_apply16c_drop(x1, self._chan_stats(x1), hi, lo, prec, w, b, drop, eps, G, act, mean_rstd=mean_rstd, film=film,
                                 film_off=film_off, film_bstride=film_bstride)
        elif film is not None:
            ops.gn_apply16c_film(x1, self._chan_stats(x1), hi, lo, prec, w, b, film, film_off, film_bstride, eps, G, act, mean_rstd=mean_rstd)
        else:
            ops.gn_apply16c(x1, self._chan_stats(x1), x2, None if x2 is None else self._chan_stats(x2), hi, lo, prec, w, b, eps, G, act,
                            x2_bmod, raw, mean_rstd=mean_rstd)

    def _gn_next(self, norm: nn.GroupNorm, act: int, planes, mr, only: bool) -> tuple:
        return (norm.weight, norm.bias, norm.eps, norm.num_groups, act, planes if self.precision.npass == 3 else planes[0], mr, only)

    def _asked(self, key: tuple, ask):
        hit = self._consts.get(key)
        if hit is None:
            hit = self._consts[key] = ask()
        return hit

    def _coop_for(self, site: str, B, H, W, co, prec):
        if not (prec.npass == 1 and co == 128 and 256 < H * W <= 1024 and B * H * W // 256 >= ops.device_cus() and not os.environ.get("STEDM_NO_GN_COOP")):
            return None
        ck = (site, B)
        words = self._coop_bufs.get(ck)
        if words is None:
            words = self._coop_bufs[ck] = torch.zeros((B, 4, 128, 2), dtype=torch.int64, device=self._coop_state.device)
        if not self._coop_advanced:
            ops.step_advance(self._coop_state, 1)
            self._coop_advanced = True
        return words, self._coop_state

    def _cat_plane(self, B, H, W, co, next_cat):
        self._catpp ^= 1
        return self._buf(f"cat16.{self._catpp}.{B}x{H}x{W}x{next_cat}", (B, H, W, next_cat), torch.int16)

    def _res(self, tag: str, rb: ResBlock, x1, x2, emb_all, emb_off, emb_bstride, x2_bmod=0, want16=False, next_cat=None, next_norm=None):
        prec = self.precision
        B, H, W, _ = x1.shape
        co = rb.out_channels
        pk = self._packed[id(rb.in_layers[2])]
        has_skip = not isinstance(rb.skip_connection, nn.Identity)
        xres = x1
        if rb.updown:
            assert x2 is None and not has_skip
            H, W = (2 * H, 2 * W) if rb.up else (H // 2, W // 2)
            a16, _, mr = self._keep(rb.in_layers[0], x1, (B, H, W, x1.shape[-1]))
            xres = self._buf(f"xr.{B}x{H}x{W}x{x1.shape[-1]}", (B, H, W, x1.shape[-1]))
            self._gn_site(rb.in_layers[0], 1, x1, hi=a16[0], lo=a16[1], prec=prec, mean_rstd=mr, resample=2 if rb.up else 1, xr=xres)
        h = self._buf(tag + ".h" if self._tape is not None else f"h.{B}x{H}x{W}x{co}", (B, H, W, co))
        self._last_h = h
        h16_next = gn_next = None
        if has_skip:
            a16, x16 = self._norm16(rb.in_layers[0], 1, x1, x2, x2_bmod, want_raw=True)
        elif not rb.updown:
            a16 = self._norm16(rb.in_layers[0], 1, x1, x2, x2_bmod)
        ws = self._splitk_ws_res(B * H * W * co)
        gn2 = rb.out_layers[0]
        film = rb.use_scale_shift_norm
        drop = None
        if self._tape is not None and self._drop_live(rb):
            drop = self._drop_used[id(rb)] = self._drop_args(rb)
        if not film and drop is None and ((prec.npass == 1 and (self._tape is None or prec.mm_dtype == BF16)) or (prec.npass == 3 and self._tape is None)):
            h16_next, _, mr2 = self._keep(gn2, h, (B, H, W, co), "g16")
            gn_next = self._gn_next(gn2, 1, h16_next, mr2, self._tape is None)
        done1 = False
        coop = self._coop_for(tag, B, H, W, co, prec) if gn_next is not None and self._tape is None else None
        coop_runs = coop is not None
        if (gn_next is not None and self._tape is None and prec.npass == 1 and prec.mm_dtype == BF16 and H * W > 256 and B >= 8 and not coop_runs and
                not os.environ.get("STEDM_NO_H16ONLY") and ops.gn_apply16c_x16_ok(co, 0, gn2.num_groups)):
            hraw = self._buf(f"h16raw.{B}x{H}x{W}x{co}", (B, H, W, co), torch.int16)
            kw1 = dict(prec=prec, src16=a16, bias=pk.bias, emb=emb_all, emb_offset=emb_off, emb_bstride=emb_bstride, w_frag=pk.frag,
                       chan_stats=self._cs_new(h), ws=ws, w_frag16=pk.frag16, out16=(hraw, None), out16_stride=co, cout=co)
            if self._asked(("h16only", id(rb), B, H, W), lambda: bool(ops.conv_igemm(None, pk.hi, pk.lo, None, query_rs=True, **kw1))):
                ops.conv_igemm(None, pk.hi, pk.lo, None, **kw1)
                ops.gn_apply16c_x16(co, self._cs[h.data_ptr()], None, None, h16_next[0], hraw, prec, gn2.weight, gn2.bias, gn2.eps, gn2.num_groups, 1)
                done1 = True
        if not done1:
            kw1 = dict(prec=prec, bias=pk.bias, emb=None if film else emb_all, emb_offset=emb_off, emb_bstride=emb_bstride, w_frag=pk.frag,
                       chan_stats=self._cs_new(h), ws=ws, w_frag16=pk.frag16, gn_next=gn_next, coop=coop)
            self._in_conv(tag, rb, pk, a16, x1.shape[-1], x2_bmod if x2 is not None else 0, h, kw1)
        if film or drop is not None:
            h16_next, _, mr2 = self._keep(gn2, h, (B, H, W, co), "g16")
            self._gn_site(gn2, 1, h, hi=h16_next[0], lo=h16_next[1], prec=prec, mean_rstd=mr2, film=emb_all if film else None, film_off=emb_off,
                          film_bstride=emb_bstride, drop=drop)
        out = self._buf(tag + ".out", (B, H, W, co))
        pk2 = self._packed[id(rb.out_layers[3])]
        o16 = None
        if want16:
            o16 = self._planes(B, H, W, co, "up16")
            self._raw16[out.data_ptr()] = o16
        gnn, npl, coop2 = None, None, None
        if next_norm is not None and self._tape is None and o16 is None and next_cat is None and not os.environ.get("STEDM_NO_NEXT_GN"):
            npl = self._planes(B, H, W, co)
            gnn = self._gn_next(*next_norm, npl, None, False)
            coop2 = self._coop_for(tag + ".c2", B, H, W, co, prec)

        def filed():
            if gnn is not None:
                self._pre16[out.data_ptr()] = (id(next_norm[0]), next_norm[1], npl)
            return out
        if has_skip:
            ps = self._packed[id(rb.skip_connection)]
            h16 = h16_next if h16_next is not None else self._norm16(rb.out_layers[0], 1, h)
            kw = dict(prec=prec, src16=h16, bias=pk2.bias, w_frag=pk2.frag, chan_stats=self._cs_new(out), ws=ws, out16=o16, w_frag16=pk2.frag16)
            kwf = dict(kw, skip=(x16[0], ps.frag, ps.bias, ps.frag16))
            fused = self._asked(("fuse", id(rb), B, H, W), lambda: bool((pk2.frag is not None or pk2.frag16 is not None) and ps.frag is not None and
                                                                        ops.conv_igemm(None, pk2.hi, pk2.lo, out, query_fused=True, **kwf)))
            if fused and next_cat is not None and o16 is None:
                rawn = self._cat_plane(B, H, W, co, next_cat)
                kwc = dict(kwf, out16=(rawn, None), out16_stride=next_cat, cout=co)
                if self._asked(("fusecat", id(rb), B, H, W, next_cat), lambda: bool(ops.conv_igemm(None, pk2.hi, pk2.lo, None, query_fused=True, **kwc))):
                    ops.conv_igemm(None, pk2.hi, pk2.lo, None, **kwc)
                    self._x16[out.data_ptr()] = (rawn, co)
                    return out
            if fused and o16 is not None and self._tape is None and prec.npass == 1:
                kw16 = dict(kwf, chan_stats=None)
                if self._asked(("fuse16", id(rb), B, H, W), lambda: bool(ops.conv_igemm(None, pk2.hi, pk2.lo, None, query_fused=True, **kw16))):
                    self._cs.pop(out.data_ptr(), None)
                    ops.conv_igemm(None, pk2.hi, pk2.lo, None, **kw16)
                    return out
            if fused:
                ops.conv_igemm(None, pk2.hi, pk2.lo, out, gn_next=gnn, **kwf)
            else:
                ops.conv_igemm(None, ps.hi, ps.lo, out, prec=prec, ks=1, src16=x16, bias=ps.bias, w_frag=ps.frag, ws=ws,
                               w_frag16=ps.frag16 if prec.npass == 3 else None)
                ops.conv_igemm(None, pk2.hi, pk2.lo, out, res=out, gn_next=gnn, **kw)
            return filed()
        assert x2 is None
        h16 = h16_next if h16_next is not None else self._norm16(rb.out_layers[0], 1, h)
        if next_cat is not None and o16 is None:
            rawn = self._cat_plane(B, H, W, co, next_cat)
            kwc = dict(prec=prec, src16=h16, bias=pk2.bias, res=xres, w_frag=pk2.frag, chan_stats=self._cs_new(out), ws=ws, w_frag16=pk2.frag16,
                       out16=(rawn, None), out16_stride=next_cat, cout=co)
            if self._asked(("rescat", id(rb), B, H, W, next_cat), lambda: bool(ops.conv_igemm(None, pk2.hi, pk2.lo, None, query_rs=True, **kwc))):
                ops.conv_igemm(None, pk2.hi, pk2.lo, None, **kwc)
                self._x16[out.data_ptr()] = (rawn, co)
                return out
        ops.conv_igemm(None, pk2.hi, pk2.lo, out, prec=prec, src16=h16, bias=pk2.bias, res=xres, w_frag=pk2.frag,
                       chan_stats=self._cs_new(out), ws=ws, out16=o16, w_frag16=pk2.frag16, gn_next=gnn, coop=coop2)
        return filed()

    def _in_conv(self, tag: str, rb: ResBlock, pk, a16, c1: int, x2_bmod: int, h, kw) -> None:
        plan = self._shared_skip(rb, pk, a16, c1, x2_bmod, h, kw)
        if plan is None:
            ops.conv_igemm(None, pk.hi, pk.lo, h, src16=a16, **kw)
            return
        seam, P, P2 = plan
        if P2 is not None:
            shared, rest = self._skip_kw(pk, a16, kw, seam, P.shape[0], P2.view(-1), res=P2[0], res2=P2[1])
            n = ops.conv_igemm(None, pk.hi, pk.lo, P, partials=True, **shared)
            assert n == 2, n
        else:
            shared, rest = self._skip_kw(pk, a16, kw, seam, P.shape[0], kw["ws"], res=P)
            ops.conv_igemm(None, pk.hi, pk.lo, P, **shared)
        ops.conv_igemm(None, pk.hi, pk.lo, h, **rest)

    @staticmethod
    def _skip_kw(pk, a16, kw, seam: int, Bs: int, ws, **res):
        return (dict(prec=kw["prec"], src16=(a16[0][:Bs, :, :, seam:], None), w_frag=pk.frag, w_frag16=pk.frag16, ws=ws),
                dict(kw, src16=(a16[0][:, :, :, :seam], None), res_bmod=Bs, **res))

    def _shared_skip(self, rb: ResBlock, pk, a16, c1: int, x2_bmod: int, h, kw):
        Bd, H, W, co = h.shape
        if (self.cfg_shared_skip is False or self._tape is not None or self.precision.npass != 1 or x2_bmod <= 0 or Bd != 2 * x2_bmod or
                a16[0].shape[0] != Bd or not a16[0].is_contiguous()):
            return None
        key = ("sskip", id(rb), Bd, H, W, self.cfg_shared_skip, self.cfg_skip_partials)

        def ask():
            C = a16[0].shape[-1]
            cpg = C // rb.in_layers[0].num_groups
            seam = -(-(-(-c1 // cpg) * cpg) // 32) * 32
            if (C - seam) // 32 > 1 and ((C - seam) // 32) % 2:
                seam += 32
            if not (32 <= seam <= C - 32 and (pk.frag is not None or pk.frag16 is not None)):
                return 0
            P = self._buf(f"sskip.P.{x2_bmod}x{H}x{W}x{co}", (x2_bmod, H, W, co))
            shared, rest = self._skip_kw(pk, a16, kw, seam, x2_bmod, kw["ws"], res=P)
            if not (ops.conv_igemm(None, pk.hi, pk.lo, P, query_rs=True, **shared) and ops.conv_igemm(None, pk.hi, pk.lo, h, query_rs=True, **rest) and
                    (self.cfg_shared_skip or self._shared_skip_rule(Bd, H, W, co, C, seam))):
                return 0
            two = (self.cfg_skip_partials is True and kw["ws"] is not None and
                   ops.conv_igemm(None, pk.hi, pk.lo, P, partials=True, query_rs=True, **shared) == 2)
            if two:
                P2 = self._buf(f"sskip.P2.{x2_bmod}x{H}x{W}x{co}", (2, x2_bmod, H, W, co))
                shared, rest = self._skip_kw(pk, a16, kw, seam, x2_bmod, P2.view(-1), res=P2[0], res2=P2[1])
                two = (ops.conv_igemm(None, pk.hi, pk.lo, P, partials=True, query_rs=True, **shared) == 2 and
                       bool(ops.conv_igemm(None, pk.hi, pk.lo, h, query_rs=True, **rest)))
            self._consts[("sskip2",) + key[1:]] = bool(two)
            return seam
        seam = self._asked(key, ask)
        if not seam:
            return None
        P2 = self._buf(f"sskip.P2.{x2_bmod}x{H}x{W}x{co}", (2, x2_bmod, H, W, co)) if self._consts[("sskip2",) + key[1:]] else None
        return seam, self._buf(f"sskip.P.{x2_bmod}x{H}x{W}x{co}", (x2_bmod, H, W, co)), P2

    @staticmethod
    def _shared_skip_rule(Bd: int, H: int, W: int, co: int, C: int, seam: int) -> bool:
        cus = ops.device_cus()

        def fills(b):
            tiles_m = -(-b * H * W // 256) if H * W >= 256 else -(-b // (256 // (H * W)))
            return tiles_m * -(-co // 128) * 4 >= cus * 3
        if not fills(Bd):
            return False
        return (C - seam) // 32 >= (14 if fills(Bd // 2) else 32)

    def _replicate(self, h, nrep: int):
        h2 = self._buf("mid.rep", (nrep * h.shape[0],) + tuple(h.shape[1:]))
        cs1 = self._cs.get(h.data_ptr())
        cs2 = self._cs_new(h2, nslab=cs1.shape[1]) if cs1 is not None else None
        h2.view((nrep,) + tuple(h.shape)).copy_(h.unsqueeze(0).expand((nrep,) + tuple(h.shape)))
        if cs2 is not None:
            cs2.view((nrep,) + tuple(cs1.shape)).copy_(cs1.unsqueeze(0).expand((nrep,) + tuple(cs1.shape)))
        return h2

    def _front_ws(self, nel: int) -> torch.Tensor:
        return self._buf("sfront.ws", ((16 if nel <= (1 << 20) else (4 if nel <= (1 << 22) else (2 if nel <= (1 << 23) else 1))) * nel,))

    def _front_kw(self, tag: str, rb: ResBlock, x1, next_norm):
        prec = self.precision
        B, H, W, _ = x1.shape
        Bd, co = 2 * B, rb.out_channels
        pk, pk2 = self._packed[id(rb.in_layers[2])], self._packed[id(rb.out_layers[3])]
        h = self._buf(f"h.{Bd}x{H}x{W}x{co}", (Bd, H, W, co))
        out = self._buf(tag + ".out", (Bd, H, W, co))
        h16 = self._planes(Bd, H, W, co, "g16")
        gnn = npl = coop2 = None
        if next_norm is not None and not os.environ.get("STEDM_NO_NEXT_GN"):
            npl = self._planes(Bd, H, W, co)
            gnn = self._gn_next(*next_norm, npl, None, False)
            coop2 = self._coop_for(tag + ".c2", Bd, H, W, co, prec)
        part = dict(prec=prec, w_frag=pk.frag, w_frag16=pk.frag16, ws=self._front_ws(B * H * W * co), partials=True)
        fin = dict(prec=prec, ws_bmod=B, bias=pk.bias, gn_next=self._gn_next(rb.out_layers[0], 1, h16, None, True))
        tail = dict(prec=prec, src16=h16, bias=pk2.bias, res=x1, res_bmod=B, w_frag=pk2.frag, ws=self._splitk_ws_res(Bd * H * W * co), w_frag16=pk2.frag16,
                    gn_next=gnn, coop=coop2)
        return pk, pk2, h, out, npl, part, fin, tail

    def _shared_front(self, tag: str, rb: ResBlock, x1shape, next_norm) -> bool:
        B, H, W, C = x1shape
        if (self.cfg_shared_front is False or self._tape is not None or self.precision.npass != 1 or not isinstance(rb.skip_connection, nn.Identity) or
                rb.out_channels != C or rb.use_scale_shift_norm or self._drop_live(rb)):
            return False
        key = ("sfront", id(rb), 2 * B, H, W, self.cfg_shared_front)

        def ask():
            pk, pk2, h, out, npl, part, fin, tail = self._front_kw(tag, rb, self._buf("mid.a.0.out", x1shape), next_norm)
            if (pk.frag is not None or pk.frag16 is not None) and C % 4 == 0 and (self.cfg_shared_front or self._shared_front_rule(2 * B, H, W, C)):
                a16 = self._planes(B, H, W, C)
                n = ops.conv_igemm(None, pk.hi, pk.lo, self._buf(f"h.{B}x{H}x{W}x{C}", (B, H, W, C)), src16=a16, query_rs=True, **part)
                if n and ops.conv_igemm(None, pk2.hi, pk2.lo, out, chan_stats=self._cs_new(out), query_rs=True, **tail):
                    return int(n)
            return 0
        return bool(self._asked(key, ask))

    @staticmethod
    def _shared_front_rule(Bd: int, H: int, W: int, co: int) -> bool:
        cus = ops.device_cus()
        tiles_m = -(-Bd * H * W // 256) if H * W >= 256 else -(-Bd // (256 // (H * W)))
        return tiles_m * -(-co // 128) * 2 >= cus

    def _res_front(self, tag: str, rb: ResBlock, x1, style_all, next_norm):
        B, H, W, C = x1.shape
        pk, pk2, h, out, npl, part, fin, tail = self._front_kw(tag, rb, x1, next_norm)
        a16 = self._norm16(rb.in_layers[0], 1, x1)
        n = ops.conv_igemm(None, pk.hi, pk.lo, self._buf(f"h.{B}x{H}x{W}x{C}", (B, H, W, C)), src16=a16, **part)
        self._last_h = h
        ops.conv_finish(part["ws"], n, h, emb=style_all, emb_bstride=style_all.shape[1], chan_stats=self._cs_new(h), **fin)
        ops.conv_igemm(None, pk2.hi, pk2.lo, out, chan_stats=self._cs_new(out), **tail)
        if npl is not None:
            self._pre16[out.data_ptr()] = (id(next_norm[0]), next_norm[1], npl)
        return out

    def _attn(self, tag: str, ab: AttentionBlock, x):
        prec = self.precision
        B, H, W, Cc = x.shape
        pq = self._packed[id(ab.qkv)]
        pp = self._packed[id(ab.proj_out)]
        out = self._buf(tag + ".out", (B, H, W, Cc))
        ch = Cc // ab.num_heads
        if prec.npass == 1 and self._tape is None and ch in (16, 32, 64, 128):
            qkv16 = self._planes(B, H, W, 3 * Cc, "qkv16")
            ops.conv_igemm(None, pq.hi, pq.lo, None, prec=prec, ks=1, src16=self._norm16(ab.norm, 0, x), bias=pq.bias, w_frag=pq.frag,
                           out16=qkv16)
            a16 = self._planes(B, H, W, Cc, "attn16")
            ops.attn_legacy16(qkv16[0].view(B, H * W, 3 * Cc), a16[0], ab.num_heads, prec, **ab.order_kw())
            ops.conv_igemm(None, pp.hi, pp.lo, out, prec=prec, ks=1, src16=a16, bias=pp.bias, res=x, w_frag=pp.frag,
                           chan_stats=self._cs_new(out), ws=self._splitk_ws(out.numel()))
            return out
        qkv = self._buf(tag + ".qkv", (B, H, W, 3 * Cc))
        ops.conv_igemm(None, pq.hi, pq.lo, qkv, prec=prec, ks=1, src16=self._norm16(ab.norm, 0, x), bias=pq.bias, w_frag=pq.frag,
                       w_frag16=pq.frag16 if prec.npass == 3 else None)
        a = self._buf(tag + ".a", (B, H, W, Cc))
        ops.attn_legacy(qkv.view(B, H * W, 3 * Cc), a.view(B, H * W, Cc), ab.num_heads, **ab.order_kw())
        if self._tape is not None:
            self._tape.append(("attn", ab, x, qkv, a, out))
        ops.conv_igemm(None, pp.hi, pp.lo, out, prec=prec, ks=1, src16=self._norm16(None, 0, a), bias=pp.bias, res=x, w_frag=pp.frag,
                       chan_stats=self._cs_new(out), w_frag16=pp.frag16 if prec.npass == 3 else None)
        return out

    def _down(self, ltag: str, layer: Downsample, h):
        B, H, W, _ = h.shape
        out = self._buf(ltag + ".out", (B, H // 2, W // 2, layer.out_channels))
        if self._tape is not None:
            self._tape.append(("down", layer, h, out))
        if not layer.use_conv:
            ops.avgpool2x2(h, out, self._cs_new(out))
            return out
        pk = self._packed[id(layer.op)]
        ps2 = self._packed.get((id(layer.op), "s2d"))
        if H % 2 == 0 and W % 2 == 0 and not ops.conv3x3_tiles_ok(H // 2, W // 2):
            return ops.conv_igemm(None, pk.hi, pk.lo, out, prec=self.precision, mode=CONV_DOWN, src16=self._norm16(None, 0, h), bias=pk.bias,
                                  chan_stats=self._cs_new(out))
        elif ps2 is not None and H % 2 == 0 and W % 2 == 0 and (H // 2) * (W // 2) >= 16:
            C = h.shape[-1]
            planes = self._buf(f"s2d16.{B}x{H}x{W}x{C}", (B, H // 2, W // 2, 4 * C), torch.int16)
            planes_lo = self._buf(f"s2d16lo.{B}x{H}x{W}x{C}", (B, H // 2, W // 2, 4 * C), torch.int16) if self.precision.npass == 3 else None
            ws = self._splitk_ws(out.numel())
            kw2 = dict(prec=self.precision, mode=CONV_S2D, src16=(planes, planes_lo), bias=ps2.bias, w_frag=ps2.frag, w_frag16=ps2.frag16, ws=ws)
# ... 221 lines not shown
```

Measured before the change: 169.1 steps/s.

## Add K-pair variant of 3x3 register-streamed conv splitting K across wave pairs

```diff
diff --git a/include/stedm_hip.h b/include/stedm_hip.h
--- a/include/stedm_hip.h
+++ b/include/stedm_hip.h
@@ -144,6 +144,7 @@
   int32_t res_bmod;
   const float* res2;
   int32_t ws_bmod;
+  int32_t k_pair;
 } stedm_conv_args;
 int stedm_conv_igemm(const stedm_conv_args* args, void* stream);
 int stedm_conv_fused_skip_ok(const stedm_conv_args* args);
diff --git a/stedm_amd/_lib.py b/stedm_amd/_lib.py
--- a/stedm_amd/_lib.py
+++ b/stedm_amd/_lib.py
@@ -41,7 +41,7 @@
         ("out16_stride", C.c_int32),
         ("gn_coop", C.c_void_p), ("gn_coop_epoch", C.c_void_p), ("gn_coop_tmo", C.c_void_p),
         ("src16_cstride", C.c_int32), ("k_chan0", C.c_int32), ("w_cin", C.c_int32), ("res_bmod", C.c_int32),
-        ("res2", C.c_void_p), ("ws_bmod", C.c_int32),
+        ("res2", C.c_void_p), ("ws_bmod", C.c_int32), ("k_pair", C.c_int32),
     ]
 
 
diff --git a/stedm_amd/csrc/conv_dma_bf16_p1.hip b/stedm_amd/csrc/conv_dma_bf16_p1.hip
--- a/stedm_amd/csrc/conv_dma_bf16_p1.hip
+++ b/stedm_amd/csrc/conv_dma_bf16_p1.hip
@@ -4,7 +4,7 @@
 int conv_dma_pick_bf16_p1(ConvParams& p, hipStream_t st, bool dry) {
   int rc = conv_rs_pick<__bf16>(p, st, dry);
   if (rc >= 0 || dry || p.a.src16b_hi || p.a.mode == STEDM_CONV_S2D || p.a.qkv_q || p.a.ln_gamma) return rc;
-  if (p.a.src16_cstride || p.a.k_chan0 || p.a.w_cin || p.a.res_bmod || p.a.res2 || p.partials || p.a.out16_stride) return rc;
+  if (p.a.src16_cstride || p.a.k_chan0 || p.a.w_cin || p.a.res_bmod || p.a.res2 || p.partials || p.a.out16_stride || p.a.k_pair == 1) return rc;
   rc = dma9_pick<__bf16>(p, st);
   return rc >= 0 ? rc : dma_pick<1, __bf16>(p, st);
 }
diff --git a/stedm_amd/csrc/conv_dma_f16_p1.hip b/stedm_amd/csrc/conv_dma_f16_p1.hip
--- a/stedm_amd/csrc/conv_dma_f16_p1.hip
+++ b/stedm_amd/csrc/conv_dma_f16_p1.hip
@@ -4,7 +4,7 @@
 int conv_dma_pick_f16_p1(ConvParams& p, hipStream_t st, bool dry) {
   int rc = conv_rs_pick<_Float16>(p, st, dry);
   if (rc >= 0 || dry || p.a.src16b_hi || p.a.mode == STEDM_CONV_S2D || p.a.qkv_q || p.a.ln_gamma) return rc;
-  if (p.a.src16_cstride || p.a.k_chan0 || p.a.w_cin || p.a.res_bmod || p.a.res2 || p.partials || p.a.out16_stride) return rc;
+  if (p.a.src16_cstride || p.a.k_chan0 || p.a.w_cin || p.a.res_bmod || p.a.res2 || p.partials || p.a.out16_stride || p.a.k_pair == 1) return rc;
   rc = dma9_pick<_Float16>(p, st);
   return rc >= 0 ? rc : dma_pick<1, _Float16>(p, st);
 }
diff --git a/stedm_amd/csrc/conv_igemm_dma.hip b/stedm_amd/csrc/conv_igemm_dma.hip
--- a/stedm_amd/csrc/conv_igemm_dma.hip
+++ b/stedm_amd/csrc/conv_igemm_dma.hip
@@ -31,6 +31,7 @@
     set_error("conv_igemm(dma): the register-streamed kernel does not run this problem, and no other kernel knows a K window, res_bmod / res2, the partials-only form or out16_stride (see stedm_conv_rs_ok)");
     return 1;
   }
+  if (rc < 0 && a.k_pair == 1) { set_error("conv_igemm(dma): k_pair = 1 requires the K-pair form and this problem does not admit it (see stedm_conv_rs_ok)"); return 1; }
   if (rc < 0 && a.src16b_hi) { set_error("conv_igemm(dma): no kernel runs this fused skip problem (see stedm_conv_fused_skip_ok)"); return 1; }
   if (rc < 0) { set_error("conv_igemm(dma): no tile configuration fits (Hin=%d Win=%d mode=%d Cin=%d)", a.Hin, a.Win, a.mode, p.Cin); return 1; }
   return rc;
diff --git a/stedm_amd/csrc/conv_rs.inc b/stedm_amd/csrc/conv_rs.inc
--- a/stedm_amd/csrc/conv_rs.inc
+++ b/stedm_amd/csrc/conv_rs.inc
@@ -310,13 +310,14 @@
 #undef LDSR
 }
 
-template <typename T, int WM, int KIND, bool FUSE = false, bool P3 = false>
+template <typename T, int WM, int KIND, bool FUSE = false, bool P3 = false, bool KP = false>
 __global__ void __launch_bounds__((16 / WM + 2) * 64) conv_rs_kernel(const ConvParams p) {
+  static_assert(!KP || (KIND == RS_3X3M && WM == 4 && !P3), "the K-pair form belongs to the single-product 16x16x32 3x3 kind");
   static_assert(!FUSE || KIND == RS_3X3 || KIND == RS_3X3M, "the fused skip phase belongs to the 3x3 kinds");
   static_assert(!P3 || ((KIND == RS_3X3M || KIND == RS_1X1M || KIND == RS_SUBM) && !FUSE), "the 3-product form exists for the plain 16x16x32 kinds");
   static_assert(KIND != RS_1X1M || (P3 && !FUSE && WM == 4), "RS_1X1M is a 3-product kind");
   static_assert(KIND != RS_SUBM || (!FUSE && WM == 4), "RS_SUBM: plain epilogues, one compute wave per SIMD");
-  constexpr int NCW = 16 / WM, NT = (NCW + 2) * 64, BMT = 256;
+  constexpr int NCW = 16 / WM, NT = (NCW + 2) * 64, BMT = KP ? 128 : 256;
   constexpr bool NPERS = KIND == RS_1X1N, IS1X1 = KIND == RS_1X1 || NPERS, SUBM = KIND == RS_SUBM, SUBPIX = KIND == RS_SUB || SUBM;
   constexpr bool G1 = KIND == RS_1X1M;
   constexpr bool M16 = KIND == RS_3X3M || G1 || SUBM;
@@ -336,7 +337,7 @@
   const int nai = (p.NP + PPI - 1) / PPI;
   const int a_plane = nai * 1024;
   const int a_half = NPL * a_plane + (M16 ? 32 : 0);
-  const int a_buf = P3 ? 2 * a_half : ((FUSE && NPL * a_plane < 32768) ? 32768 : a_half);
+  const int a_buf = KP ? ((FUSE && 2 * a_half < 32768) ? 32768 : 2 * a_half) : (P3 ? 2 * a_half : ((FUSE && NPL * a_plane < 32768) ? 32768 : a_half));
   const int pl_skew = (KIND == RS_3X3M || SUBM) ? 16 : 0;
   int* sM = reinterpret_cast<int*>(smem);
   int* sMb = sM + BMT;
@@ -370,10 +371,10 @@
   const int m0 = tile_m * BMT, n0 = tile_n * BN;
   const int nchunks_all = p.Cin / BKC;
   const int nchunks_w = p.w_cin / BKC;
-  const int nsteps = split ? nchunks_all / p.ksplit : nchunks_all;
+  const int nsteps = KP ? nchunks_all / 2 : (split ? nchunks_all / p.ksplit : nchunks_all);
   const int cbeg = kz * nsteps;
   const int nsteps2_all = FUSE ? a.cb / 64 : 0;
-  const int nsteps2 = split ? nsteps2_all / p.ksplit : nsteps2_all;
+  const int nsteps2 = KP ? nsteps2_all / 2 : (split ? nsteps2_all / p.ksplit : nsteps2_all);
   const int c2beg = split ? kz * nsteps2 : 0;
   STAMP(0);
 
@@ -446,7 +447,7 @@
     const uint16_t* a_hi = reinterpret_cast<const uint16_t*>(a.src16_hi);
     const uint16_t* zero16 = reinterpret_cast<const uint16_t*>(g_zero_page);
     const int nslots = (nai + 1 - aw) / 2;
-    constexpr int MAXS = IS1X1 ? 16 : 13;
+    constexpr int MAXS = IS1X1 ? 16 : (KP ? 7 : 13);
     const uint16_t* asrc[MAXS];
     const int lpos = lane / CPP, lphys = lane % CPP;
     const long lo_delta = P3 ? reinterpret_cast<const uint16_t*>(a.src16_lo) - a_hi : 0;
@@ -466,6 +467,7 @@
           for (int pl = 0; pl < NPL; ++pl) {
             GLDS16(asrc[k] + (cbeg * NPL + pl) * (BROW / 2), sA + pl * (a_plane + pl_skew) + (aw + 2 * k) * 1024);
             if (P3) GLDS16(LO_SRC(k) + (cbeg * NPL + pl) * (BROW / 2), sA + a_half + pl * (a_plane + pl_skew) + (aw + 2 * k) * 1024);
+            if (KP) GLDS16(asrc[k] + ((cbeg + nsteps) * NPL + pl) * (BROW / 2), sA + a_half + pl * (a_plane + pl_skew) + (aw + 2 * k) * 1024);
           }
         }
       }
@@ -481,6 +483,7 @@
           if (k < nslots) {
             GLDS16(asrc[k] + c0, dsta + pl * (a_plane + pl_skew) + (aw + 2 * k) * 1024);
             if (P3) GLDS16(LO_SRC(k) + c0, dsta + a_half + pl * (a_plane + pl_skew) + (aw + 2 * k) * 1024);
+            if (KP) GLDS16(asrc[k] + c0 + nsteps * NPL * (BROW / 2), dsta + a_half + pl * (a_plane + pl_skew) + (aw + 2 * k) * 1024);
           }
         }
       }
@@ -501,10 +504,11 @@
     for (int c = 1; c < 3; ++c)
       if (c < nsteps) { issue_a(c); early[c] = true; }
     __syncthreads();
-    int aoff2[FUSE ? 16 : 1];
+    constexpr int NK2 = FUSE ? BMT / 16 : 0;
+    int aoff2[FUSE ? NK2 : 1];
     if (FUSE) {
 #pragma unroll
-      for (int k = 0; k < 16; ++k) {
+      for (int k = 0; k < NK2; ++k) {
         const int ml = (aw + 2 * k) * 8 + (lane >> 3);
         const int logical = (lane & 7) ^ ((ml >> 1) & 7);
         const int m = sM[ml];
@@ -517,10 +521,11 @@
       unsigned char* dsta = sA + ringpos * a_buf;
       const int c0 = (c2beg + c2) * 64;
 #pragma unroll
-      for (int k = 0; k < (FUSE ? 16 : 0); ++k) {
+      for (int k = 0; k < NK2; ++k) {
         const int o = aoff2[k];
         const uint16_t* sh = o >= 0 ? b_hi + o + c0 : zero16 + (-o - 1) + c0;
         GLDS16(sh, dsta + (aw + 2 * k) * 1024);
+        if (KP) GLDS16(sh + nsteps2 * 64, dsta + BMT * 128 + (aw + 2 * k) * 1024);
       }
     };
     auto issue_any = [&](int chunk) {
@@ -537,7 +542,7 @@
         default: WAIT_VM(0); break;
       }
     };
-    auto wait_all_but = [&](int chunk) { wait_keep((FUSE && chunk >= nsteps) ? 16 : nslots * NPL); };
+    auto wait_all_but = [&](int chunk) { wait_keep((FUSE && chunk >= nsteps) ? 16 : nslots * NPL * (KP ? 2 : 1)); };
     {
       if (!early[0]) issue_any(0);
       if (ntot > 1 && !early[1]) issue_any(1);
@@ -559,11 +564,12 @@
     __syncthreads();
     STAMP(1);
     STAMPC(2);
-    const int wm = wave >> 1, wn = wave & 1;
+    const int wm = KP ? 0 : wave >> 1, wn = wave & 1;
+    const int kzw = KP ? wave >> 1 : 0;
     const int r = lane & 31, h = lane >> 5;
     const unsigned voff = lane * 16;
     int abuf = 0;
-    const unsigned A0 = (unsigned)(uintptr_t)sA;
+    const unsigned A0 = (unsigned)(uintptr_t)sA + (unsigned)(kzw * a_half);
     if constexpr (M16) {
       const int r16 = lane & 15;
       unsigned aofs[1][8];
@@ -578,7 +584,7 @@
       for (int t = 0; t < NS; ++t)
         tapd[t] = G1 ? 0u : (SUBM ? (unsigned)((t >> 1) * p.PW + (t & 1)) * 32u : (unsigned)((t / 3) * p.PW + (t % 3)) * 32u);
       const unsigned char* wq = reinterpret_cast<const unsigned char*>(a.w_frag16) +
-                                (((((size_t)parity * p.tiles_n + tile_n) * nchunks_w + cbeg) * NS) * 8 + wn * 4) * 1024;
+                                (((((size_t)parity * p.tiles_n + tile_n) * nchunks_w + cbeg + kzw * nsteps) * NS) * 8 + wn * 4) * 1024;
       f32x4 acc[8][4];
 #pragma unroll
       for (int i = 0; i < 8; ++i)
@@ -601,13 +607,14 @@
             aofs2[sl][f] = ml * 128 + ((((unsigned)(4 * sl) + (unsigned)(lane >> 4)) ^ ((ml >> 1) & 7)) << 4);
           }
         const unsigned tapd2[2] = {0u, 0u};
-        const unsigned char* wq2 = reinterpret_cast<const unsigned char*>(a.w_frag_b16) + ((((size_t)tile_n * nsteps2_all + c2beg) * 2) * 8 + wn * 4) * 1024;
-        rs_phase16<T, 2, 2, false>(acc, aofs2, tapd2, A0, a_buf, abuf, nsteps2, wq2, voff);
+        const unsigned char* wq2 = reinterpret_cast<const unsigned char*>(a.w_frag_b16) + ((((size_t)tile_n * nsteps2_all + c2beg + kzw * nsteps2) * 2) * 8 + wn * 4) * 1024;
+        const unsigned A02 = (unsigned)(uintptr_t)sA + (unsigned)(kzw * (BMT * 128));
+        rs_phase16<T, 2, 2, false>(acc, aofs2, tapd2, A02, a_buf, abuf, nsteps2, wq2, voff);
       }
       __syncthreads();
       STAMP(3);
       STAMPC(7);
-      if (!STEDM_DBG(p.dbg, 64)) {
+      if (!STEDM_DBG(p.dbg, 64) && (!KP || kzw == 1)) {
         const int g4 = lane >> 4;
 #pragma unroll
         for (int i = 0; i < 8; ++i)
@@ -617,6 +624,20 @@
 #pragma unroll
             for (int e = 0; e < 4; ++e) dst[e * SST] = acc[i][j][e];
           }
+      }
+      if constexpr (KP) {
+        __syncthreads();
+        if (kzw == 0) {
+          const int g4 = lane >> 4;
+#pragma unroll
+          for (int i = 0; i < 8; ++i)
+#pragma unroll
+            for (int j = 0; j < 4; ++j) {
+              float* dst = sStage + (i * 16 + g4 * 4) * SST + wn * 64 + j * 16 + r16;
+#pragma unroll
+              for (int e = 0; e < 4; ++e) dst[e * SST] = acc[i][j][e] + dst[e * SST];
+            }
+        }
       }
     } else {
     unsigned aofs[TAPS][WM];
@@ -813,6 +834,7 @@
     }
   }
   if (is_loader) __syncthreads();
+  if (KP && is_loader) __syncthreads();
   if STEDM_DBG(p.dbg, 64) return;
   __syncthreads();
   STAMP(5);
@@ -1387,10 +1409,11 @@
   return 0;
 }
 
-template <typename T, int WM, int KIND, bool FUSE = false, bool P3 = false>
+template <typename T, int WM, int KIND, bool FUSE = false, bool P3 = false, bool KP = false>
 static int conv_rs_try(ConvParams& p, const ConvParams& q, hipStream_t st, bool dry = false) {
   constexpr size_t LDS_MAX = 160 * 1024;
-  constexpr int BMT = 256;
+  constexpr int BMT = KP ? 128 : 256;
+  if (KP && (q.ksplit >= 2 || q.partials || q.a.gn_coop)) return -1;
   constexpr bool G1 = KIND == RS_1X1M;
   constexpr bool SUBK = KIND == RS_SUB || KIND == RS_SUBM;
   constexpr bool M16 = KIND == RS_3X3M || G1 || KIND == RS_SUBM;
@@ -1398,7 +1421,7 @@
   constexpr int PPI = K1 ? 8 : (G1 ? 16 : 32), NPL = (SUBK || KIND == RS_3X3M) ? 2 : 1, NTAB = (KIND == RS_3X3 || KIND == RS_3X3M) ? 9 : 4;
   if ((KIND == RS_3X3M || G1) && q.a.mode != STEDM_CONV_S1) return -1;
   const size_t nai = (q.NP + PPI - 1) / PPI;
-  if ((nai + 1) / 2 > (K1 ? 16 : 13)) return -1;
+  if ((nai + 1) / 2 > (K1 ? 16 : (KP ? 7 : 13))) return -1;
   bool stats = q.a.chan_stats != nullptr;
   if (stats && (K1 || G1) && !(BMT % q.HWout == 0 || q.HWout % BMT == 0)) stats = false;
   const bool s2d = SUBK && q.a.mode == STEDM_CONV_S2D;
@@ -1409,6 +1432,7 @@
   if (stats && SUBK && !s2d && q.a.chan_nslab == 0) stats = false;
   if (stats && q.ksplit >= 2 && !fine_ok && q.a.chan_nslab != 0 && (HWo + 255) / 256 != q.a.chan_nslab) stats = false;
   size_t a_buf = NPL * nai * 1024 + (M16 ? 32 : 0);
+  if (KP) a_buf *= 2;
   if (FUSE && a_buf < 32768) a_buf = 32768;
   if (P3) a_buf *= 2;
   const size_t ring = (P3 ? 3 : 4) * a_buf;
@@ -1429,6 +1453,7 @@
     return -1;
   if (q.a.ln_gamma && (KIND != RS_1X1 || q.tiles_n != 1 || q.ksplit >= 2)) return -1;
   if (!q.a.out && q.a.chan_stats && !stats) return -1;
+  if (KP && q.a.chan_stats && (!stats || BMT % q.HWout != 0)) return -1;
   if (q.a.out16_stride && (KIND == RS_1X1N || P3)) return -1;
   const bool kwin = q.a.src16_cstride || q.a.k_chan0 || q.a.w_cin;
   if ((kwin || q.a.res_bmod || q.a.res2 || q.partials) && !((KIND == RS_3X3 || KIND == RS_3X3M) && !FUSE && !P3)) return -1;
@@ -1461,7 +1486,7 @@
     const int cpg = (a_.gn_out16 && a_.gn_groups > 0) ? a_.cout / a_.gn_groups : 0;
     const int nt = p.HWout / BMT;
     static const bool off = getenv("STEDM_NO_GN_COOP") != nullptr;
-    if (!p.gn_tile && !off && cpg > 0 && stats && q.ksplit < 2 && (KIND == RS_3X3 || KIND == RS_3X3M) && !FUSE && !P3 && p.HWout % BMT == 0 && nt >= 2 && nt <= 4 &&
+    if (!p.gn_tile && !off && !KP && cpg > 0 && stats && q.ksplit < 2 && (KIND == RS_3X3 || KIND == RS_3X3M) && !FUSE && !P3 && p.HWout % BMT == 0 && nt >= 2 && nt <= 4 &&
         a_.cout == 128 && p.tiles_n == 1 && p.xcd_m == 0 && !p.whole && cpg % 4 == 0 && 128 % cpg == 0 && 256 % a_.gn_groups == 0 && a_.out && !a_.out16_hi && !a_.act_out &&
         a_.gn_coop && a_.gn_coop_epoch && a_.gn_coop_tmo && (size_t)lds + 4 * 128 * 2 * sizeof(float) <= LDS_MAX)
       p.gn_coop = nt;
@@ -1479,7 +1504,7 @@
     if (q.a.w_frag) kp.a.w_frag = reinterpret_cast<const unsigned char*>(q.a.w_frag) + (size_t)q.a.k_chan0 * 9 * 256;
     if (q.a.w_frag16) kp.a.w_frag16 = reinterpret_cast<const unsigned char*>(q.a.w_frag16) + (size_t)q.a.k_chan0 * 9 * 256;
   }
-  auto k = conv_rs_kernel<T, WM, KIND, FUSE, P3>;
+  auto k = conv_rs_kernel<T, WM, KIND, FUSE, P3, KP>;
   const size_t lds_launch = lds + (p.gn_coop ? (size_t)4 * 128 * 2 * sizeof(float) : 0);
   static size_t lds_set = 0;
   if (lds_launch > lds_set) {
@@ -1499,6 +1524,12 @@
   if (stats) p.stats_done = 1;
   if (p.gn_tile || p.gn_coop) p.gn_done = 1;
   return 0;
+}
+
+static bool conv_k_pair_rule(const ConvParams& p, const ConvParams& q, const int cus) {
+  const long t256 = (long)q.tiles_m * q.tiles_n;
+  const long tm128 = p.HWout <= 128 ? (p.a.B + 128 / p.HWout - 1) / (128 / p.HWout) : (p.M + 127) / 128;
+  return p.HWout <= 128 && t256 * 4 < (long)cus * 3 && tm128 * q.tiles_n * 4 >= (long)cus * 3;
 }
 
 template <typename T>
@@ -1512,6 +1543,7 @@
   if (s2d && !sp) return -1;
   const bool k3 = a.ks == 3 && p.taps == 9 && p.Cin % 16 == 0, k1 = a.ks == 1 && p.Cin % 64 == 0;
   if (!k3 && !k1 && !sp) return -1;
+  if (a.k_pair == 1 && !(k3 && a.mode == STEDM_CONV_S1)) return -1;
   if (a.qkv_q && (!k1 || fuse || !a.w_frag)) return -1;
   if (a.ln_gamma && (!k1 || fuse || !a.w_frag || a.cout > 128)) return -1;
   static int cus = 0;
@@ -1539,6 +1571,21 @@
   const bool m16 = k3 && a.mode == STEDM_CONV_S1 && a.w_frag16 && p.Cin % 32 == 0 && p.Cin >= 256 && (!fuse || a.w_frag_b16);
   if (!a.w_frag && !m16 && !subm) return -1;
   if (fuse && !m16 && !a.w_frag_b) return -1;
+  {
+    const int nch = p.Cin / 32;
+    bool ok = m16 && (!fuse || (a.cb / 64) % 2 == 0) && !p.partials && a.k_pair != 2 && nch % 2 == 0 && nch / 2 >= 4 &&
+              (p.HWout <= 128 ? 128 % p.HWout == 0 : (128 % p.Wout == 0 && p.HWout % 128 == 0));
+    if (ok && a.k_pair == 0) ok = conv_k_pair_rule(p, q, cus);
+    if (ok) {
+      ConvParams q2 = p;
+      if (conv_geometry(q2, 128, false)) {
+        q2.ksplit = 0;
+        const int rc = fuse ? conv_rs_try<T, 4, RS_3X3M, true, false, true>(p, q2, st, dry) : conv_rs_try<T, 4, RS_3X3M, false, false, true>(p, q2, st, dry);
+        if (rc >= 0) return rc;
+      }
+    }
+    if (a.k_pair == 1) return -1;
+  }
   if ((long)q.tiles_m * q.tiles_n * (sp ? 4 : 1) * 4 < (long)cus * 3) {
     const int ks = k3 ? pick_split((long)q.tiles_m * q.tiles_n, p.Cin / (m16 ? 32 : 16), 1, fuse ? a.cb / 64 : 0)
                  : (k1 && !fuse)      ? pick_split((long)q.tiles_m * q.tiles_n, p.Cin / 64)
diff --git a/stedm_amd/ops.py b/stedm_amd/ops.py
--- a/stedm_amd/ops.py
+++ b/stedm_amd/ops.py
@@ -479,15 +479,16 @@
                skip: Optional[Tuple[torch.Tensor, torch.Tensor, Optional[torch.Tensor]]] = None, query_fused: bool = False, query_rs: bool = False,
                ws: Optional[torch.Tensor] = None, pad_br: bool = False, w_frag16: Optional[torch.Tensor] = None,
                gn_next: Optional[tuple] = None, qkv_planes: Optional[tuple] = None, ln_after: Optional[tuple] = None, coop: Optional[tuple] = None,
-               out16_stride: int = 0, cout: Optional[int] = None, res_bmod: int = 0, res2: Optional[torch.Tensor] = None, partials: bool = False):
+               out16_stride: int = 0, cout: Optional[int] = None, res_bmod: int = 0, res2: Optional[torch.Tensor] = None, partials: bool = False,
+               k_pair=None):
     if src16 is not None and src1 is None and ks == 3 and mode in (CONV_S1, CONV_DOWN, CONV_UP) and not out16_stride:
         _, H_, W_, _ = src16[0].shape
         Ho_, Wo_ = ((H_ - 1) // 2 + 1, (W_ - 1) // 2 + 1) if mode == CONV_DOWN else ((2 * H_, 2 * W_) if mode == CONV_UP else (H_, W_))
         if not conv3x3_tiles_ok(Ho_, Wo_):
             if query_fused or query_rs:
                 return False
-            if not src16[0].is_contiguous() or res_bmod or res2 is not None or partials:
-                raise _lib.StedmHipError("conv_igemm: a K window / res_bmod belongs to the tiled register-streamed kernel; this output grid takes the im2col form")
+            if not src16[0].is_contiguous() or res_bmod or res2 is not None or partials or k_pair is True:
+                raise _lib.StedmHipError("conv_igemm: a K window / res_bmod / k_pair belongs to the tiled register-streamed kernel; this output grid takes the im2col form")
             return _conv3x3_generic(src16, w_hi, w_lo, out, prec=prec, mode=mode, scale=scale, shift=shift, act=act, bias=bias, emb=emb,
                                     emb_offset=emb_offset, emb_bstride=emb_bstride, res=res, act_out=act_out, out16=out16, chan_stats=chan_stats,
                                     skip=skip, ws=ws, gn_next=gn_next)
@@ -594,6 +595,7 @@
                        w_frag16.shape[-5] * 32 if w_frag16 is not None else wplanes.shape[-1] if wplanes is not None else cs)
             assert w_frag is None or w_frag16 is None or w_frag.shape[-5] * 16 == w_frag16.shape[-5] * 32
     a.res_bmod = int(res_bmod)
+    a.k_pair = 0 if k_pair is None else (1 if k_pair else 2)
     if res_bmod:
         assert res is not None and res.is_contiguous() and res.dtype == torch.float32 and B % res_bmod == 0 and res.shape[0] >= res_bmod
     if res2 is not None:
@@ -614,6 +616,8 @@
     a.out = _ptr(out)
     a.cout = oshape[-1]
     a.npass, a.mm_dtype = prec.npass, prec.mm_dtype
+    if k_pair == "prefer" and not (src16 is not None and lib().stedm_conv_rs_ok(C.byref(a))):
+        a.k_pair = 0
     if lazy is not None and lazy._val is None:
         if src16 is None or (w_frag is None and w_frag16 is None) or prec.npass != 1 or not lib().stedm_conv_rs_ok(C.byref(a)):
             w_hi, w_lo = lazy.get()
diff --git a/stedm_amd/unet.py b/stedm_amd/unet.py
--- a/stedm_amd/unet.py
+++ b/stedm_amd/unet.py
@@ -257,6 +257,7 @@
         self.cfg_shared_skip: Optional[bool] = None
         self.cfg_shared_front: Optional[bool] = None
         self.cfg_skip_partials: Optional[bool] = None
+        self.conv_k_pair: Optional[bool] = None
 
     def convert_to_fp16(self):
         pass
@@ -557,10 +558,15 @@
         return (norm.weight, norm.bias, norm.eps, norm.num_groups, act, planes if self.precision.npass == 3 else planes[0], mr, only)
 
     def _asked(self, key: tuple, ask):
+        key = key + (("k_pair", self.conv_k_pair),)
         hit = self._consts.get(key)
         if hit is None:
             hit = self._consts[key] = ask()
         return hit
+
+    @property
+    def _kp(self):
+        return "prefer" if self.conv_k_pair is True else self.conv_k_pair
 
     def _coop_for(self, site: str, B, H, W, co, prec):
         if not (prec.npass == 1 and co == 128 and 256 < H * W <= 1024 and B * H * W // 256 >= ops.device_cus() and not os.environ.get("STEDM_NO_GN_COOP")):
@@ -614,14 +620,14 @@
                 not os.environ.get("STEDM_NO_H16ONLY") and ops.gn_apply16c_x16_ok(co, 0, gn2.num_groups)):
             hraw = self._buf(f"h16raw.{B}x{H}x{W}x{co}", (B, H, W, co), torch.int16)
             kw1 = dict(prec=prec, src16=a16, bias=pk.bias, emb=emb_all, emb_offset=emb_off, emb_bstride=emb_bstride, w_frag=pk.frag,
-                       chan_stats=self._cs_new(h), ws=ws, w_frag16=pk.frag16, out16=(hraw, None), out16_stride=co, cout=co)
+                       chan_stats=self._cs_new(h), ws=ws, w_frag16=pk.frag16, out16=(hraw, None), out16_stride=co, cout=co, k_pair=self._kp)
             if self._asked(("h16only", id(rb), B, H, W), lambda: bool(ops.conv_igemm(None, pk.hi, pk.lo, None, query_rs=True, **kw1))):
                 ops.conv_igemm(None, pk.hi, pk.lo, None, **kw1)
                 ops.gn_apply16c_x16(co, self._cs[h.data_ptr()], None, None, h16_next[0], hraw, prec, gn2.weight, gn2.bias, gn2.eps, gn2.num_groups, 1)
                 done1 = True
         if not done1:
             kw1 = dict(prec=prec, bias=pk.bias, emb=None if film else emb_all, emb_offset=emb_off, emb_bstride=emb_bstride, w_frag=pk.frag,
-                       chan_stats=self._cs_new(h), ws=ws, w_frag16=pk.frag16, gn_next=gn_next, coop=coop)
+                       chan_stats=self._cs_new(h), ws=ws, w_frag16=pk.frag16, gn_next=gn_next, coop=coop, k_pair=self._kp)
             self._in_conv(tag, rb, pk, a16, x1.shape[-1], x2_bmod if x2 is not None else 0, h, kw1)
         if film or drop is not None:
             h16_next, _, mr2 = self._keep(gn2, h, (B, H, W, co), "g16")
@@ -646,7 +652,7 @@
         if has_skip:
             ps = self._packed[id(rb.skip_connection)]
             h16 = h16_next if h16_next is not None else self._norm16(rb.out_layers[0], 1, h)
-            kw = dict(prec=prec, src16=h16, bias=pk2.bias, w_frag=pk2.frag, chan_stats=self._cs_new(out), ws=ws, out16=o16, w_frag16=pk2.frag16)
+            kw = dict(prec=prec, src16=h16, bias=pk2.bias, w_frag=pk2.frag, chan_stats=self._cs_new(out), ws=ws, out16=o16, w_frag16=pk2.frag16, k_pair=self._kp)
             kwf = dict(kw, skip=(x16[0], ps.frag, ps.bias, ps.frag16))
             fused = self._asked(("fuse", id(rb), B, H, W), lambda: bool((pk2.frag is not None or pk2.frag16 is not None) and ps.frag is not None and
                                                                         ops.conv_igemm(None, pk2.hi, pk2.lo, out, query_fused=True, **kwf)))
@@ -675,13 +681,13 @@
         if next_cat is not None and o16 is None:
             rawn = self._cat_plane(B, H, W, co, next_cat)
             kwc = dict(prec=prec, src16=h16, bias=pk2.bias, res=xres, w_frag=pk2.frag, chan_stats=self._cs_new(out), ws=ws, w_frag16=pk2.frag16,
-                       out16=(rawn, None), out16_stride=next_cat, cout=co)
+                       out16=(rawn, None), out16_stride=next_cat, cout=co, k_pair=self._kp)
             if self._asked(("rescat", id(rb), B, H, W, next_cat), lambda: bool(ops.conv_igemm(None, pk2.hi, pk2.lo, None, query_rs=True, **kwc))):
                 ops.conv_igemm(None, pk2.hi, pk2.lo, None, **kwc)
                 self._x16[out.data_ptr()] = (rawn, co)
                 return out
         ops.conv_igemm(None, pk2.hi, pk2.lo, out, prec=prec, src16=h16, bias=pk2.bias, res=xres, w_frag=pk2.frag,
-                       chan_stats=self._cs_new(out), ws=ws, out16=o16, w_frag16=pk2.frag16, gn_next=gnn, coop=coop2)
+                       chan_stats=self._cs_new(out), ws=ws, out16=o16, w_frag16=pk2.frag16, gn_next=gnn, coop=coop2, k_pair=self._kp)
         return filed()
 
     def _in_conv(self, tag: str, rb: ResBlock, pk, a16, c1: int, x2_bmod: int, h, kw) -> None:
@@ -701,7 +707,7 @@
 
     @staticmethod
     def _skip_kw(pk, a16, kw, seam: int, Bs: int, ws, **res):
-        return (dict(prec=kw["prec"], src16=(a16[0][:Bs, :, :, seam:], None), w_frag=pk.frag, w_frag16=pk.frag16, ws=ws),
+        return (dict(prec=kw["prec"], src16=(a16[0][:Bs, :, :, seam:], None), w_frag=pk.frag, w_frag16=pk.frag16, ws=ws, k_pair=kw.get("k_pair")),
                 dict(kw, src16=(a16[0][:, :, :, :seam], None), res_bmod=Bs, **res))
 
     def _shared_skip(self, rb: ResBlock, pk, a16, c1: int, x2_bmod: int, h, kw):
@@ -778,7 +784,7 @@
         part = dict(prec=prec, w_frag=pk.frag, w_frag16=pk.frag16, ws=self._front_ws(B * H * W * co), partials=True)
         fin = dict(prec=prec, ws_bmod=B, bias=pk.bias, gn_next=self._gn_next(rb.out_layers[0], 1, h16, None, True))
         tail = dict(prec=prec, src16=h16, bias=pk2.bias, res=x1, res_bmod=B, w_frag=pk2.frag, ws=self._splitk_ws_res(Bd * H * W * co), w_frag16=pk2.frag16,
-                    gn_next=gnn, coop=coop2)
+                    gn_next=gnn, coop=coop2, k_pair=self._kp)
         return pk, pk2, h, out, npl, part, fin, tail
 
     def _shared_front(self, tag: str, rb: ResBlock, x1shape, next_norm) -> bool:
```

Result: no change. 170.7 steps/s (median of 6 runs) (+0.9%).
